# wzf2000/GAMER

Measured on AMD Instinct MI355X. Metric: train-step sequences/sec, Qwen3Multi SMB decoder, his_len=100, higher is better.
Workload: dtype f32 tensors/accumulators, products = 3 x fp16 pieces (split3)

## Files before the change

### gamer_amd/_lib.py

```python
from __future__ import annotations

import ctypes as C
import os
import re
from typing import Optional

import torch

_HERE = os.path.dirname(os.path.abspath(__file__))
LIB_PATH = os.path.join(_HERE, "lib", "libgamer_hip.so")
if os.environ.get("GAMER_LIB_PATH"):
    LIB_PATH = os.path.abspath(os.environ["GAMER_LIB_PATH"])
HEADER_PATH = os.path.join(os.path.dirname(_HERE), "include", "gamer_hip.h")

_lib: Optional[C.CDLL] = None

c_void_p, c_int, c_float, c_int64, c_uint64 = C.c_void_p, C.c_int, C.c_float, C.c_int64, C.c_uint64


class GemmDesc(C.Structure):
    _fields_ = [
        ("A", c_void_p), ("a_rs", c_int64), ("a_ks", c_int64),
        ("B", c_void_p), ("b_rs", c_int64), ("b_ks", c_int64),
        ("C", c_void_p), ("ldc", c_int64),
        ("M", c_int), ("N", c_int), ("K", c_int),
        ("alpha", c_float),
        ("accumulate", c_int),
        ("groups", c_int),
        ("group_mode", c_int),
        ("group_offsets", c_void_p),
        ("strideB", c_int64), ("strideC", c_int64),
        ("kchunk", c_int),
        ("resid", c_void_p),
        ("row_map", c_void_p),
        ("p_drop", c_float),
        ("seed", c_uint64),
        ("rowdot_other", c_void_p),
        ("rowdot_out", c_void_p),
        ("rowdot_S", c_int),
        ("qk_wq", c_void_p), ("qk_wk", c_void_p),
        ("qk_eps", c_float),
        ("qk_cos", c_void_p), ("qk_sin", c_void_p),
        ("qk_bias_q", c_void_p), ("qk_bias_k", c_void_p), ("qk_bias_v", c_void_p),
        ("qk_act_idx", c_void_p),
        ("qk_pos_ids", c_void_p),
        ("qk_q_rot", c_void_p), ("qk_k_rot", c_void_p),
        ("qk_S", c_int), ("qk_nq", c_int), ("qk_nkv", c_int),
        ("b_planes", c_void_p), ("b_plane_stride", c_int64),
        ("amax_a", c_void_p), ("amax_b", c_void_p),
        ("amax_c", c_void_p), ("amax_c_col0", c_int),
        ("wgrad_ws", c_void_p), ("wgrad_ws_floats", c_int64),
        ("sw_gu", c_void_p), ("sw_ld", c_int64),
        ("group_div", c_int), ("sw_tbl", c_void_p), ("b_planes_t", c_void_p),
        ("sw_hm", c_void_p), ("sw_row_group", c_void_p),
    ]


class GemmBf16Desc(C.Structure):
    _fields_ = [
        ("A", c_void_p), ("lda", c_int64),
        ("B", c_void_p), ("ldb", c_int64),
        ("C", c_void_p), ("ldc", c_int64),
        ("M", c_int), ("N", c_int), ("K", c_int),
        ("accumulate", c_int),
        ("groups", c_int),
        ("group_mode", c_int),
        ("group_offsets", c_void_p),
        ("strideB", c_int64), ("strideC", c_int64),
        ("kchunk", c_int),
        ("resid", c_void_p),
        ("row_map", c_void_p),
        ("p_drop", c_float),
        ("seed", c_uint64),
        ("rowdot_other", c_void_p),
        ("rowdot_out", c_void_p),
        ("rowdot_S", c_int),
        ("qk_wq", c_void_p), ("qk_wk", c_void_p), ("qk_eps", c_float),
        ("qk_cos", c_void_p), ("qk_sin", c_void_p),
        ("qk_bias_q", c_void_p), ("qk_bias_k", c_void_p), ("qk_bias_v", c_void_p),
        ("qk_act_idx", c_void_p), ("qk_pos_ids", c_void_p),
        ("qk_q_rot", c_void_p), ("qk_k_rot", c_void_p),
        ("qk_S", c_int), ("qk_nq", c_int), ("qk_nkv", c_int),
        ("sw_gu", c_void_p), ("sw_ld", c_int64),
        ("wgrad_ws", c_void_p), ("wgrad_ws_floats", c_int64),
    ]


P, I, F, L, U = c_void_p, c_int, c_float, c_int64, c_uint64

_SIGNATURES = {
    "gamer_router_fwd": [P, P, P, P, I, I, I, I, I, I, P, P, P, P, P, P, P, P, P, P, P, P],
    "gamer_expert_lists": [P, I, I, I, P, P, P, P, P],
    "gamer_causal_prep": [P, I, I, P, P, P, P, P, P],
    "gamer_session_prep": [P, P, P, I, I, I, I, P, P, P, P, P, P, P],
    "gamer_moe_router_prep": [P, P, P, I, P, I, I, I, I, I, I, I, P, P, P, P, P, P, P, P, P],
    "gamer_embedding_fwd": [P, P, I, I, I, P, P],
    "gamer_embedding_bwd": [P, P, I, I, I, I, P, P],
    "gamer_embedding_bwd_ordered": [P, P, I, I, I, I, P, P, L, P],
    "gamer_embedding_bwd_ordered_ws_bytes": [I, I, I],
    "gamer_rmsnorm_fwd": [P, P, I, I, F, P, P, I, P],
    "gamer_rmsnorm_bwd": [P, P, P, I, P, I, I, F, I, P, P, I, P, P, F, U, P],
    "gamer_colsum_reduce": [P, I, I, I, P, P],
    "gamer_colsum_reduce_batched": [P, L, I, I, I, P, I, P],
    "gamer_rowtable_fwd": [P, P, P, I, I, P, I, I, P],
    "gamer_rowtable_bwd": [P, I, I, P, P, I, I, I, P, P, L, P],
    "gamer_gemm_f32": [C.POINTER(GemmDesc), P],
    "gamer_gemm_f32_split": [C.POINTER(GemmDesc), c_int, P],
    "gamer_split3_guard": [I],
    "gamer_gemm_bf16": [C.POINTER(GemmBf16Desc), P],
    "gamer_cast_params_bf16": [P, P, P, P, I, I, P],
    "gamer_attn_fwd_bf16": [P, I, P, I, P, I, P, P, I, I, I, I, F, F, U, P, P, P, P, P, P, P],
    "gamer_attn_bwd_bf16": [P, I, P, I, P, I, P, P, P, P, P, I, I, I, I, F, F, U, P, P, I, P, I, P, I, P, I, P, P, P, P],
    "gamer_session_spans": [P, P, P, P, P, I, I, I, I, P, P, P, P, P, P, P, P, P],
    "gamer_qknorm_rope_fwd": [P, I, I, I, I, P, P, F, P, P, P, P, P, P, P, P, P, P],
    "gamer_qknorm_rope_bwd": [P, P, P, I, I, I, I, P, P, F, P, P, P, P, P, I, P, P, P, P, P, P, P, P, L, P],
    "gamer_attn_row_order": [P, I, I, P, P, P, P],
    "gamer_attn_fwd": [P, I, P, I, P, I, P, P, P, P, I, I, I, I, F, F, U, P, P, P, P, P, I, P, P],
    "gamer_attn_bwd": [P, I, P, I, P, I, P, P, P, P, P, P, P, I, I, I, I, F, F, U, P, P, I, P, I, P, I, P, P, P, P, P, I, P],
    "gamer_split3_planes": [P, P, L, L, P],
    "gamer_absmax_f32": [P, I, L, I, I, L, P, P],
    "gamer_absmax_multi_f32": [P, P, I, P, P],
    "gamer_split2h_planes_multi": [P, P, I, P, P, P],
    "gamer_amax_sink": [P, P],
    "gamer_amax_sink3": [P, P, P],
    "gamer_attn_split_amax": [P, P, P, P],
    "gamer_attn_fwd_split": [P, I, P, I, P, I, P, P, P, I, I, I, I, F, F, U, P, P, P, P, P, I, P, P],
    "gamer_attn_bwd_split": [P, I, P, I, P, I, P, P, P, P, P, P, P, I, I, I, I, F, F, U, P, P, I, P, I, P, I, P, P, P, I, P, P, P],
    "gamer_residual_dropout_fwd": [P, P, P, I, I, F, U, P, P],
    "gamer_residual_dropout_bwd": [P, P, I, I, F, U, P, P],
    "gamer_swiglu_fwd": [P, P, L, F, U, P, P],
    "gamer_swiglu_bwd": [P, P, P, L, F, U, P],
    "gamer_swiglu_fwd_ld": [P, L, I, I, F, U, P, P],
    "gamer_swiglu_bwd_ld": [P, L, I, I, P, F, U, P],
    "gamer_swiglu_fwd_ld_tbl": [P, L, I, I, F, U, P, P, P, P],
    "gamer_swiglu_bwd_ld_tbl": [P, L, I, I, P, F, U, P, P, P],
    "gamer_silu_fwd_ld": [P, L, I, I, F, U, P, P],
    "gamer_silu_bwd_ld": [P, L, I, I, P, F, U, P],
    "gamer_router_position_table": [P, L, P, I, P],
    "gamer_inject_table_fwd": [P, P, L, I, I, I, I, I, P, P],
    "gamer_segment_colsum_ws_floats": [I, I, I],
    "gamer_segment_colsum": [P, L, I, I, P, I, P, L, P, P],
    "gamer_inject_table_bwd": [P, P, P, L, I, I, I, I, I, P, P, P, P],
    "gamer_silu_gate_fwd": [P, P, L, P, P, F, U, P],
    "gamer_silu_gate_bwd": [P, P, P, L, P, P, F, U, P],
    "gamer_check_labels": [P, L, I, I, P, P],
    "gamer_ce_fwd": [P, I, P, I, I, I, F, I, P, P, P, P, P],
    "gamer_ce_bwd": [P, I, P, I, I, I, F, I, P, P, F, F, P, P],
    "gamer_sumsq": [P, L, P, I, P],
    "gamer_adamw": [P, P, P, P, L, L, F, F, F, F, F, I, F, F, P, I, P, P],
    "gamer_fill_f32": [P, L, F, P],
    "gamer_bias_act_fwd": [P, P, I, I, I, P, P],
    "gamer_bias_act_bwd": [P, P, I, I, I, P, P, I, P],
    "gamer_layernorm_fwd": [P, P, P, P, I, I, F, P, P, P, P, P],
    "gamer_layernorm_bwd": [P, P, P, P, P, I, I, P, P, P, I, P],
    "gamer_attn_dense_fwd": [P, I, P, I, P, I, P, P, I, I, I, I, F, F, U, P, I, P, P],
    "gamer_attn_dense_bwd": [P, I, P, I, P, I, P, P, I, I, I, I, F, F, U, P, P, I, P, P, I, P, I, P, I, P],
    "gamer_reload_env": [],
    "gamer_split2h_transpose_multi": [P, P, I, P, P],
    "gamer_trie_logprobs": [P, L, P, P, P, P, P, I, I, P, P],
    "gamer_trie_advance": [P, P, P, P, P, I, P, P],
    "gamer_kv_append": [P, I, P, I, P, P, I, I, I, I, I, P],
    "gamer_attn_decode": [P, I, P, I, P, I, P, P, P, I, I, I, I, P, I, I, I, I, I, F, P, P],
    "gamer_attn_decode_split": [P, I, P, I, P, I, P, P, P, I, I, I, I, P, I, I, I, I, I, F, P, P, P, P],
    "gamer_catalog_ws_bytes": [I, I, I, I],
    "gamer_catalog_ce_fwd": [P, L, P, I, I, P, I, I, P, P, P, P, P, L, P],
    "gamer_catalog_ce_bwd": [P, L, P, I, I, P, I, I, P, P, P, F, P, P, L, P, L, P],
    "gamer_catalog_topk": [P, L, P, I, I, P, I, I, I, I, I, P, P, P, L, P],
    "gamer_catalog_ce_bias_fwd": [P, L, P, I, I, P, I, I, P, P, P, P, P, P, L, P],
    "gamer_catalog_ce_bias_bwd": [P, L, P, I, I, P, I, I, P, P, P, P, F, P, P, L, P, P, L, P],
    "gamer_catalog_topk_bias": [P, L, P, I, I, P, I, I, P, I, I, I, P, P, P, L, P],
    "gamer_cloze_mask_ws_bytes": [I, I],
    "gamer_cloze_mask": [P, P, I, I, F, F, L, I, U, P, P, P, P, P, P, P, L, P],
    "gamer_embedding_bwd_large_ws_bytes": [I, I, I],
    "gamer_embedding_bwd_large": [P, P, I, I, I, I, P, P, L, P],
    "gamer_position_bwd_ws_floats": [I, I, I],
    "gamer_position_bwd": [P, I, I, I, P, P, L, P],
    "gamer_seq_embed_ln_fwd": [P, P, I, P, I, I, I, P, P, F, F, U, P, P, P, P, P],
    "gamer_gru_gates_floats": [I, I, I],
    "gamer_gru_fwd": [P, P, P, I, I, I, P, P, P],
    "gamer_gru_bwd": [P, P, P, P, P, I, I, I, P, P, P],
    "gamer_mbs_mix_fwd": [P, P, I, I, I, P, P],
    "gamer_mbs_mix_bwd": [P, P, P, I, I, I, P, P, P],
    "gamer_mbs_attn_fwd": [P, I, P, I, P, I, P, P, P, P, P, I, I, I, I, I, I, F, F, U, P, I, P, P],
    "gamer_mbs_attn_bwd": [P, I, P, I, P, I, P, P, P, P, P, I, I, I, I, I, I, F, F, U, P, P, I, P, P, I, P, I, P, I, P, P, P, I, P],
    "gamer_mbs_bias_fold": [P, P, I, I, I, I, P, P],
    "gamer_mbs_gate_mix_fwd": [P, I, P, P, I, I, I, P, P, P],
    "gamer_mbs_gate_mix_bwd": [P, P, P, I, I, I, P, P, I, P],
    "gamer_pbat_attn_fwd": [P, P, P, P, P, P, I, P, P, P, P, P, P, P, P, P, P, P, P, P, P, I, I, I, I, I, F, F, U, P, P, I, P, P, P, P],
    "gamer_pbat_attn_bwd": [P, P, P, P, P, P, I, P, P, P, P, P, P, P, P, P, P, P, P, P, P, I, I, I, I, I, F, F, U, P, P, P, P, I, P, P, P, P, P, P, I, P, P, P, P, I, P, P],
    "gamer_wass_rows_fwd": [P, P, I, I, P, P, P],
    "gamer_wass_rows_bwd": [P, P, P, P, I, I, P, P, P],
    "gamer_wass_table_fwd": [P, P, I, I, P, P, P],
    "gamer_wass_table_bwd": [P, P, P, P, I, I, P, P, P],
    "gamer_rvq_ws_floats": [I],
    "gamer_rvq_fwd": [P, L, P, P, P, I, I, I, I, I, P, P, P, P, P, P, P, P],
    "gamer_rvq_bwd": [P, P, P, P, I, I, I, P, P, F, P, P, P],
    "gamer_msa_linear_fwd": [P, I, P, I, P, I, P, P, P, P, P, I, I, I, I, I, F, F, U, P, I, P, P],
    "gamer_msa_linear_bwd": [P, I, P, I, P, I, P, P, P, P, P, I, I, I, I, I, F, F, U, P, I, P, P, I, P, I, P, I, P, I, P],
    "gamer_seq_mix_fwd": [P, I, P, I, P, I, P, P, I, I, I, P, P],
    "gamer_seq_mix_bwd": [P, I, P, I, P, I, P, P, I, I, I, P, P, P, P, I, P],
    "gamer_hg_build_fwd": [P, P, I, I, I, I, I, P, P, P],
    "gamer_hg_build_bwd": [P, P, P, P, P, I, I, I, I, I, P, P],
    "gamer_hg_conv_fwd": [P, P, I, I, I, P, P],
    "gamer_hg_conv_bwd": [P, P, P, I, I, I, P, P, P],
    "gamer_hg_readout_fwd": [P, P, P, I, I, I, I, I, I, I, P, P],
    "gamer_hg_readout_bwd": [P, P, P, I, I, I, I, I, I, I, P, P],
    "gamer_hg_fuse_fwd": [P, P, P, L, I, P, P, P],
# ... 77 lines not shown
```

### gamer_amd/csrc/common.h

```cpp
#pragma once
#include <hip/hip_runtime.h>
#include <stdint.h>
#include <stdio.h>
#include <stdarg.h>
#include <stdlib.h>
#include <atomic>
#include <type_traits>

#include "../../include/gamer_hip.h"

namespace gamer {

void set_error(const char* fmt, ...);

#define GAMER_CHECK_ARG(cond, ...)                       \
    do {                                                 \
        if (!(cond)) {                                   \
            gamer::set_error(__VA_ARGS__);               \
            return -1;                                   \
        }                                                \
    } while (0)

#define GAMER_CHECK_LAUNCH(name)                                                        \
    do {                                                                                \
// ... 129 lines not shown
AmaxSink take_amax_sink();
void disarm_attn_amax();
__device__ __forceinline__ uint32_t amax_f4(uint32_t m, const float4 v) {
    float f = __uint_as_float(m);
    f = fmaxf(fmaxf(f, fabsf(v.x)), fabsf(v.y));
    f = fmaxf(fmaxf(f, fabsf(v.z)), fabsf(v.w));
    return __float_as_uint(f);
}
constexpr int AMAX_WAYS = 16, AMAX_STRIDE = 16;
__device__ __forceinline__ uint32_t amax_read(const uint32_t* __restrict__ p) {
    uint32_t m = 0;
#pragma unroll
    for (int i = 0; i < AMAX_WAYS; ++i) m = max(m, p[AMAX_STRIDE * i]);
    return m;
}
__device__ __forceinline__ void amax_publish(uint32_t m, uint32_t* __restrict__ out, uint32_t way) {
    uint32_t* w = out + AMAX_STRIDE * (way & (AMAX_WAYS - 1));
    if (m > __hip_atomic_load(w, __ATOMIC_RELAXED, __HIP_MEMORY_SCOPE_AGENT)) atomicMax(w, m);
}
__device__ __forceinline__ void amax_block_commit(uint32_t m, uint32_t* __restrict__ out, uint32_t* __restrict__ lds4) {
    if (!out) return;
#pragma unroll
    for (int o = 32; o > 0; o >>= 1) m = max(m, (uint32_t)__shfl_xor((int)m, o, 64));
    if ((threadIdx.x & 63) == 0) lds4[threadIdx.x >> 6] = m;
    __syncthreads();
    if (threadIdx.x == 0) {
        m = max(max(lds4[0], lds4[1]), max(lds4[2], lds4[3]));
        if (m) amax_publish(m, out, blockIdx.x);
    }
}

__device__ __forceinline__ float wave_sum(float v) {
#pragma unroll
    for (int o = 32; o > 0; o >>= 1) v += __shfl_xor(v, o, 64);
    return v;
}
__device__ __forceinline__ float wave_max(float v) {
#pragma unroll
    for (int o = 32; o > 0; o >>= 1) v = fmaxf(v, __shfl_xor(v, o, 64));
    return v;
}

__device__ __forceinline__ uint32_t mix32(uint32_t x) {
    x ^= x >> 16; x *= 0x7feb352dU; x ^= x >> 15; x *= 0x846ca68bU; x ^= x >> 16;
    return x;
}
struct DropoutRng {
    uint32_t k0, k1, thr;
    float scale;
    bool on;
    __device__ __forceinline__ DropoutRng(float p, uint64_t seed) {
        on = p > 0.f;
        k0 = mix32((uint32_t)seed ^ 0x9e3779b9U);
        k1 = mix32((uint32_t)(seed >> 32) + 0x85ebca6bU);
        float t = p * 4294967296.f;
        thr = t >= 4294967040.f ? 0xffffffffU : (uint32_t)t;
        scale = on ? 1.f / (1.f - p) : 1.f;
    }
    __device__ __forceinline__ void mult4(uint32_t idx4, float (&m)[4]) const {
        if (!on) { m[0] = m[1] = m[2] = m[3] = 1.f; return; }
        const uint32_t thr16 = thr >> 16;
        const uint32_t h1 = mix32(idx4 * 0x9e3779b1U + k0);
        const uint32_t h2 = mix32(h1 ^ k1);
        m[0] = (h1 & 0xffffU) >= thr16 ? scale : 0.f;
        m[1] = (h1 >> 16) >= thr16 ? scale : 0.f;
        m[2] = (h2 & 0xffffU) >= thr16 ? scale : 0.f;
        m[3] = (h2 >> 16) >= thr16 ? scale : 0.f;
    }
    __device__ __forceinline__ float mult(uint64_t idx) const {
        if (!on) return 1.f;
        uint32_t h = mix32((uint32_t)idx ^ k0);
        h = mix32(h + (uint32_t)(idx >> 32) * 0x9e3779b1U + k1);
        return h >= thr ? scale : 0.f;
    }
};

struct AttnDropout {
    uint32_t k0, k1, thr;
    float scale;
    __device__ __forceinline__ AttnDropout(float p, uint64_t seed) {
        k0 = mix32((uint32_t)seed ^ 0x9e3779b9U) ^ mix32((uint32_t)(seed >> 32) + 0x7f4a7c15U);
        k1 = mix32(k0 + 0x632be5abU);
        const float t = p * 4294967296.f;
        thr = t >= 4294967040.f ? 0xffffffffU : (uint32_t)t;
        scale = p > 0.f ? 1.f / (1.f - p) : 1.f;
    }
    __device__ __forceinline__ uint32_t row_word(uint32_t row) const {
        return (mix32(row * 0x9e3779b1U + k0) & 0xffffffU) | 0x800001U;
    }
    __device__ __forceinline__ uint32_t key_word(uint32_t j) const { return mix32(j * 0x85ebca6bU + k1) & 0xffffffU; }
    __device__ __forceinline__ bool keep(uint32_t a, uint32_t b) const { return __umul24(a, b) >= thr; }
};

__device__ __forceinline__ float xor32_max(float v) {
    const auto sw = __builtin_amdgcn_permlane32_swap(__float_as_uint(v), __float_as_uint(v), false, false);
    return fmaxf(__uint_as_float(sw[0]), __uint_as_float(sw[1]));
}
__device__ __forceinline__ float xor32_sum(float v) {
    const auto sw = __builtin_amdgcn_permlane32_swap(__float_as_uint(v), __float_as_uint(v), false, false);
    return __uint_as_float(sw[0]) + __uint_as_float(sw[1]);
}

__device__ __forceinline__ int wave_sum_i32(int v) {
#pragma unroll
    for (int o = 32; o > 0; o >>= 1) v += __shfl_xor(v, o, 64);
    return v;
}
__device__ __forceinline__ int wave_max_i32(int v) {
#pragma unroll
    for (int o = 32; o > 0; o >>= 1) v = max(v, __shfl_xor(v, o, 64));
    return v;
}
__device__ __forceinline__ int wave_min_i32(int v) {
#pragma unroll
    for (int o = 32; o > 0; o >>= 1) v = min(v, __shfl_xor(v, o, 64));
    return v;
}

#define GAMER_DPP_ROW_REDUCE(OP, v)                                                                   \
    v = OP(v, __builtin_amdgcn_update_dpp(v, v, 0xB1, 0xf, 0xf, false));      \
    v = OP(v, __builtin_amdgcn_update_dpp(v, v, 0x4E, 0xf, 0xf, false));      \
    v = OP(v, __builtin_amdgcn_update_dpp(v, v, 0x141, 0xf, 0xf, false));         \
    v = OP(v, __builtin_amdgcn_update_dpp(v, v, 0x140, 0xf, 0xf, false));
__device__ __forceinline__ int wave_min_i32_dpp(int v) {
    GAMER_DPP_ROW_REDUCE(min, v)
    return min(min(__builtin_amdgcn_readlane(v, 0), __builtin_amdgcn_readlane(v, 16)),
               min(__builtin_amdgcn_readlane(v, 32), __builtin_amdgcn_readlane(v, 48)));
}
__device__ __forceinline__ int wave_max_i32_dpp(int v) {
    GAMER_DPP_ROW_REDUCE(max, v)
    return max(max(__builtin_amdgcn_readlane(v, 0), __builtin_amdgcn_readlane(v, 16)),
               max(__builtin_amdgcn_readlane(v, 32), __builtin_amdgcn_readlane(v, 48)));
}

__device__ __forceinline__ float row16_sum_dpp(float v) {
#define GAMER_DPP_F(ctrl) __int_as_float(__builtin_amdgcn_update_dpp(__float_as_int(v), __float_as_int(v), ctrl, 0xf, 0xf, false))
    v += GAMER_DPP_F(0xB1);
    v += GAMER_DPP_F(0x4E);
    v += GAMER_DPP_F(0x141);
    v += GAMER_DPP_F(0x140);
#undef GAMER_DPP_F
    return v;
}

__device__ __forceinline__ float sigmoid_f(float x) { return __builtin_amdgcn_rcpf(1.f + __expf(-x)); }
__device__ __forceinline__ float silu_f(float x) { return x * sigmoid_f(x); }
__device__ __forceinline__ float dsilu_f(float x) {
    const float s = sigmoid_f(x);
    return s * (1.f + x * (1.f - s));
}

bool gemm_as_eligible(const gamer_gemm_desc* d, bool a_kc, bool b_kc, const uint16_t* b_planes);
int launch_gemm_as(const gamer_gemm_desc* d, const uint16_t* b_planes, bool b_kc, hipStream_t st);
bool gemm_os_eligible(const gamer_gemm_desc* d, bool a_kc, bool b_kc, const uint16_t* b_planes);
int launch_gemm_os(const gamer_gemm_desc* d, const uint16_t* b_planes, int guard, hipStream_t st, bool fwd_t = false);
bool gemm_os_fwd_eligible(const gamer_gemm_desc* d, bool a_kc, bool b_kc);
bool gemm_wg_eligible(const gamer_gemm_desc* d, bool a_kc, bool b_kc);
int launch_gemm_wg(const gamer_gemm_desc* d, hipStream_t st);

int launch_wgrad_reduce(const float* ws, float* C, int64_t ldc, int M, int N, int groups, const int32_t* group_offsets, int K,
                        int kchunk, int64_t strideC, hipStream_t st);

}
```

### gamer_amd/csrc/gemm.hip

```cpp
#include "common.h"
#include <stdlib.h>

namespace gamer {

constexpr int BM = 128, BN = 128, BK = 32;
constexpr int GEMM_THREADS = 256;
constexpr int KC_LD = BK + 4;
constexpr int TILE_FLOATS = BM * KC_LD;
constexpr int GEMM_LDS_BYTES = 4 * TILE_FLOATS * (int)sizeof(float);

typedef float f32x16 __attribute__((ext_vector_type(16)));

constexpr int SP_KC_ROW = 80;
constexpr int SP_KC_IMG = BM * SP_KC_ROW;
constexpr int SP_RC_IMG = BK * 256;
constexpr int SP_OPERAND = 3 * SP_KC_IMG;
constexpr int SP_LDS_BYTES = 2 * SP_OPERAND;

#ifndef SP_ABLATE
#define SP_ABLATE 0
#endif
__device__ __forceinline__ uint32_t pack_hi16(uint32_t w0, uint32_t w1) { return __builtin_amdgcn_perm(w1, w0, 0x07060302u); }
__device__ __forceinline__ void split3(float x, uint32_t (&w)[3]) {
    if (SP_ABLATE & 1) { w[0] = w[1] = w[2] = __float_as_uint(x); return; }
// ... 1212 lines not shown
    const int64_t step4 = (int64_t)tiles_mn * (BM * BN) / 4;
    float4 s = make_float4(0.f, 0.f, 0.f, 0.f);
    int c = 0;
    for (; c + 4 <= c_n; c += 4) {
        const float4 a0 = src[(int64_t)c * step4], a1 = src[(int64_t)(c + 1) * step4], a2 = src[(int64_t)(c + 2) * step4],
                     a3 = src[(int64_t)(c + 3) * step4];
        s.x = (((s.x + a0.x) + a1.x) + a2.x) + a3.x; s.y = (((s.y + a0.y) + a1.y) + a2.y) + a3.y;
        s.z = (((s.z + a0.z) + a1.z) + a2.z) + a3.z; s.w = (((s.w + a0.w) + a1.w) + a2.w) + a3.w;
    }
    for (; c < c_n; ++c) {
        const float4 a0 = src[(int64_t)c * step4];
        s.x += a0.x; s.y += a0.y; s.z += a0.z; s.w += a0.w;
    }
    const int row = (tile / n_tiles) * BM + lr, col = (tile % n_tiles) * BN + lc;
    if (row < M && c_n > 0) {
        float* dst = C + (int64_t)g * strideC + (int64_t)row * ldc + col;
        const float v[4] = {s.x, s.y, s.z, s.w};
#pragma unroll
        for (int e = 0; e < 4; ++e)
            if (col + e < N) dst[e] += v[e];
    }
}

int launch_wgrad_reduce(const float* ws, float* C, int64_t ldc, int M, int N, int groups, const int32_t* group_offsets, int K,
                        int kchunk, int64_t strideC, hipStream_t st) {
    const int m_tiles = (M + BM - 1) / BM, n_tiles = (N + BN - 1) / BN;
    const int64_t rblocks = (int64_t)groups * m_tiles * n_tiles * 16;
    hipLaunchKernelGGL(wgrad_reduce_kernel, dim3((int)rblocks), dim3(256), 0, st, ws, C, ldc, M, N, m_tiles, n_tiles, groups,
                       group_offsets, K, kchunk, strideC);
    return (int)hipGetLastError();
}

__global__ void __launch_bounds__(256)
split3_planes_kernel(const float4* __restrict__ x, uint16_t* __restrict__ planes, int64_t n4, int64_t stride) {
    for (int64_t i = (int64_t)blockIdx.x * 256 + threadIdx.x; i < n4; i += (int64_t)gridDim.x * 256) {
        uint2 img[3];
        split3_quad(x[i], img);
#pragma unroll
        for (int s = 0; s < 3; ++s) *reinterpret_cast<uint2*>(planes + s * stride + 4 * i) = img[s];
    }
}

}

using namespace gamer;

extern "C" int gamer_split3_planes(const float* x, gamer_bf16* planes, int64_t n, int64_t plane_stride, void* stream) {
    GAMER_CHECK_ARG(x && planes && n > 0 && n % 4 == 0 && plane_stride >= n && plane_stride % 4 == 0 && aligned16(x) &&
                    (reinterpret_cast<uintptr_t>(planes) & 7u) == 0,
                    "gamer_split3_planes: n=%lld and plane_stride=%lld must be multiples of 4 (stride >= n), x 16-byte and planes 8-byte aligned",
                    (long long)n, (long long)plane_stride);
    const int64_t n4 = n / 4;
    int blocks = (int)((n4 + 255) / 256);
    if (blocks > 4096) blocks = 4096;
    hipLaunchKernelGGL(split3_planes_kernel, dim3(blocks), dim3(256), 0, (hipStream_t)stream, reinterpret_cast<const float4*>(x),
                       reinterpret_cast<uint16_t*>(planes), n4, plane_stride);
    GAMER_CHECK_LAUNCH("gamer_split3_planes");
    return 0;
}

extern "C" int gamer_debug_gemm_stamp(void* p) {
    unsigned long long* v = (unsigned long long*)p;
    return (int)hipMemcpyToSymbol(HIP_SYMBOL(g_gemm_stamp), &v, sizeof(v));
}

static inline bool diag_build_switches() {
    static EnvSwitch stamp("GAMER_GEMM_STAMP"), nbuf("GAMER_GEMM_NBUF");
    return stamp.is_set() || nbuf.is_set();
}
static inline bool diag_pp_switch() { static EnvSwitch pp("GAMER_GEMM_PP"); return pp.is_set(); }
static int gemm_entry(const gamer_gemm_desc* d, void* stream, int split) {
    GAMER_CHECK_ARG(d, "gamer_gemm_f32: null descriptor");
    GAMER_CHECK_ARG(d->A && d->B && d->C, "gamer_gemm_f32: null matrix pointer");
    GAMER_CHECK_ARG(d->M > 0 && d->N > 0 && d->K > 0, "gamer_gemm_f32: bad shape M=%d N=%d K=%d", d->M, d->N, d->K);
    GAMER_CHECK_ARG((d->a_rs == 1) != (d->a_ks == 1) || (d->a_rs == 1 && d->a_ks == 1 && (d->M == 1 || d->K == 1)),
                    "gamer_gemm_f32: exactly one of a_rs/a_ks must be 1 (rs=%lld ks=%lld)", (long long)d->a_rs, (long long)d->a_ks);
    GAMER_CHECK_ARG((d->b_rs == 1) != (d->b_ks == 1) || (d->b_rs == 1 && d->b_ks == 1 && (d->N == 1 || d->K == 1)),
                    "gamer_gemm_f32: exactly one of b_rs/b_ks must be 1 (rs=%lld ks=%lld)", (long long)d->b_rs, (long long)d->b_ks);
    const bool a_kc = d->a_ks == 1, b_kc = d->b_ks == 1;
    const int64_t a_ld = a_kc ? d->a_rs : d->a_ks, b_ld = b_kc ? d->b_rs : d->b_ks;
    GAMER_CHECK_ARG(a_ld % 4 == 0 && b_ld % 4 == 0 && d->ldc >= d->N,
                    "gamer_gemm_f32: leading dims must be multiples of 4 (lda=%lld ldb=%lld ldc=%lld)",
                    (long long)a_ld, (long long)b_ld, (long long)d->ldc);
    GAMER_CHECK_ARG(aligned16(d->A) && aligned16(d->B), "gamer_gemm_f32: A and B must be 16-byte aligned");
    GAMER_CHECK_ARG(d->groups >= 1 && (d->groups == 1 || d->group_offsets), "gamer_gemm_f32: groups=%d needs group_offsets", d->groups);
    GAMER_CHECK_ARG(d->strideB % 4 == 0, "gamer_gemm_f32: strideB must be a multiple of 4");
    GAMER_CHECK_ARG(d->group_mode == 0 || d->group_mode == 1, "gamer_gemm_f32: group_mode=%d", d->group_mode);

    GemmParams p;
    p.A = d->A; p.a_rs = d->a_rs; p.a_ks = d->a_ks;
    p.B = d->B; p.b_rs = d->b_rs; p.b_ks = d->b_ks;
    p.C = d->C; p.ldc = d->ldc;
    p.M = d->M; p.N = d->N; p.K = d->K;
    p.alpha = d->alpha; p.accumulate = d->accumulate;
    p.groups = d->groups; p.group_offsets = d->group_offsets;
    p.strideB = d->strideB; p.strideC = d->strideC;
    p.kchunk = d->kchunk;
    p.resid = d->resid; p.row_map = d->row_map; p.p_drop = d->p_drop; p.seed = d->seed;
    p.rowdot_other = d->rowdot_other; p.rowdot_out = d->rowdot_out; p.rowdot_S = d->rowdot_S;
    p.qk_wq = d->qk_wq; p.qk_wk = d->qk_wk; p.qk_eps = d->qk_eps; p.qk_cos = d->qk_cos; p.qk_sin = d->qk_sin;
    p.qk_bias_q = d->qk_bias_q; p.qk_bias_k = d->qk_bias_k; p.qk_bias_v = d->qk_bias_v;
    p.qk_act_idx = d->qk_act_idx; p.qk_pos_ids = d->qk_pos_ids; p.qk_q_rot = d->qk_q_rot; p.qk_k_rot = d->qk_k_rot;
    p.qk_S = d->qk_S; p.qk_nq = d->qk_nq; p.qk_nkv = d->qk_nkv;
    p.amax_a = d->amax_a; p.amax_b = d->amax_b;
    p.guard = g_split3_guard;
    p.amax_c = d->amax_c; p.amax_c_col0 = d->amax_c_col0;
    p.wgrad_ws = nullptr;
    p.sw_gu = d->sw_gu; p.sw_ld = d->sw_ld;
    p.group_div = d->group_div > 1 ? d->group_div : 1; p.sw_tbl = d->sw_tbl;
    GAMER_CHECK_ARG(d->group_div <= 1 || (d->group_mode == 0 && d->group_offsets && d->groups % d->group_div == 0),
                    "gamer_gemm_f32: group_div = %d needs group_mode 0, group_offsets and groups (%d) a multiple of it", d->group_div, d->groups);
    GAMER_CHECK_ARG(!d->sw_tbl || ((d->sw_gu || d->sw_hm) && aligned16(d->sw_tbl)),
                    "gamer_gemm_f32: sw_tbl is an option of the SwiGLU epilogues (sw_gu, sw_hm)");
    GAMER_CHECK_ARG(!d->sw_gu || (split == 3 && d->group_mode == 0 && !d->accumulate && !d->resid && !d->rowdot_out && !d->qk_q_rot &&
                                  d->alpha == 1.f && d->N % 4 == 0 && d->sw_ld >= 2 * (int64_t)d->N && d->sw_ld % 4 == 0 &&
                                  aligned16(d->sw_gu) && d->p_drop >= 0.f && d->p_drop < 1.f),
                    "gamer_gemm_f32: the SwiGLU-backward epilogue (sw_gu) is built for gamer_gemm_f32_split(terms = 3), a plain input-"
                    "gradient GEMM with alpha = 1, N %% 4 == 0, sw_ld >= 2 N (N=%d sw_ld=%lld)", d->N, (long long)d->sw_ld);
    GAMER_CHECK_ARG(!d->amax_c || (d->group_mode == 0 && !d->accumulate && !d->resid && !d->qk_q_rot && d->amax_c_col0 >= 0 &&
                                   d->amax_c_col0 % 64 == 0),
                    "gamer_gemm_f32: amax_c needs a plain or row-dot Linear-forward / input-gradient GEMM (no accumulate, residual or "
                    "q|k|v epilogue) and amax_c_col0 a multiple of 64 (amax_c_col0=%d)", d->amax_c_col0);
    GAMER_CHECK_ARG(split != 3 || (d->amax_a && d->amax_b), "gamer_gemm_f32_split: terms = 3 needs amax_a and amax_b (gamer_absmax_f32)");
    p.b_planes = (split && d->group_mode == 0) ? (const uint16_t*)d->b_planes : nullptr;
    p.b_plane_stride = d->b_plane_stride;
    GAMER_CHECK_ARG(!p.b_planes || split == 3 || ((reinterpret_cast<uintptr_t>(p.b_planes) & 7u) == 0 && d->b_plane_stride % 4 == 0 && d->b_plane_stride > 0),
                    "gamer_gemm_f32_split: b_planes must be 8-byte aligned with b_plane_stride %% 4 == 0");
    GAMER_CHECK_ARG(!p.b_planes || split != 3 || (reinterpret_cast<uintptr_t>(p.b_planes) & 15u) == 0,
                    "gamer_gemm_f32_split: terms = 3 takes b_planes as packed pieces at B's offsets (16-byte aligned)");
    if (split == 3 && p.b_planes && ((b_kc ? d->K : d->N) % 4) != 0) p.b_planes = nullptr;
    GAMER_CHECK_ARG(!d->qk_q_rot || (d->qk_k_rot && d->qk_wq && d->qk_wk && d->qk_cos && d->qk_sin && d->group_mode == 0 &&
                                     d->groups == 1 && a_kc && b_kc && !d->resid && !d->rowdot_out && !d->accumulate &&
                                     d->alpha == 1.f && d->M % BM == 0 && d->qk_nq > 0 && d->qk_nkv > 0 && d->qk_S > 0 &&
                                     d->N == (d->qk_nq + 2 * d->qk_nkv) * 64 && d->N % BN == 0 && d->ldc % 4 == 0 &&
                                     aligned16(d->C) && aligned16(d->qk_q_rot) && aligned16(d->qk_k_rot) &&
                                     (!d->qk_bias_q || (d->qk_bias_k && d->qk_bias_v && d->qk_act_idx)) &&
                                     !diag_build_switches()),
                    "gamer_gemm_f32: the q|k|v epilogue needs a Linear-forward layout, one group, M %% 128 == 0 (M=%d), "
                    "N = (nq + 2 nkv) * 64 a multiple of 128 (N=%d), alpha = 1 and no other epilogue", d->M, d->N);
    GAMER_CHECK_ARG(!d->rowdot_out || (d->rowdot_other && d->rowdot_S > 0 && d->group_mode == 0 && d->groups == 1 &&
                                       !d->resid && !d->accumulate && d->M % BM == 0 && d->N % BN == 0 &&
                                       d->M % d->rowdot_S == 0 && d->ldc % 4 == 0 && aligned16(d->rowdot_other) &&
                                       aligned16(d->C) && !diag_build_switches()),
                    "gamer_gemm_f32: the row-dot epilogue needs full 128 x 128 tiles (M=%d N=%d), one group, ldc %% 4 == 0",
                    d->M, d->N);
    GAMER_CHECK_ARG(!d->resid || (d->group_mode == 0 && !d->accumulate && a_kc && b_kc && d->ldc % 4 == 0 &&
                                  aligned16(d->resid) && aligned16(d->C) && d->p_drop >= 0.f && d->p_drop < 1.f),
                    "gamer_gemm_f32: the fused residual epilogue needs a Linear-forward layout, ldc %% 4 == 0, no accumulate");
    GAMER_CHECK_ARG(!d->sw_hm || (d->group_mode == 0 && a_kc && b_kc && !d->accumulate && !d->resid && !d->rowdot_out && !d->qk_q_rot &&
                                  !d->sw_gu && d->alpha == 1.f && d->N % 8 == 0 && d->ldc >= d->N && d->ldc % 4 == 0 && aligned16(d->sw_hm) &&
                                  aligned16(d->C) && (!d->sw_tbl || d->sw_row_group) && d->p_drop >= 0.f && d->p_drop < 1.f),
                    "gamer_gemm_f32: the SwiGLU-forward epilogue (sw_hm) needs a Linear-forward layout with N = 2 I (N=%d), alpha = 1, no other "
                    "epilogue, and sw_row_group with sw_tbl", d->N);
    if (split == 3 && gemm_as_eligible(d, a_kc, b_kc, p.b_planes)) return launch_gemm_as(d, p.b_planes, b_kc, (hipStream_t)stream);
    if (d->sw_hm) {
        gamer_gemm_desc d2 = *d;
        d2.sw_hm = nullptr; d2.sw_row_group = nullptr; d2.sw_tbl = nullptr; d2.amax_c = nullptr;
        const int rc = gemm_entry(&d2, stream, split);
        if (rc) return rc;
        if (d->amax_c) gamer_amax_sink(d->amax_c, nullptr);
        return d->sw_tbl ? gamer_swiglu_fwd_ld_tbl(d->C, d->ldc, d->M, d->N / 2, d->p_drop, d->seed, d->sw_hm, d->sw_tbl, d->sw_row_group, stream)
                         : gamer_swiglu_fwd_ld(d->C, d->ldc, d->M, d->N / 2, d->p_drop, d->seed, d->sw_hm, stream);
    }
    if (split == 3 && gemm_os_eligible(d, a_kc, b_kc, p.b_planes)) return launch_gemm_os(d, p.b_planes, g_split3_guard, (hipStream_t)stream);
    if (split == 3 && gemm_os_fwd_eligible(d, a_kc, b_kc))
        return launch_gemm_os(d, reinterpret_cast<const uint16_t*>(d->b_planes_t), g_split3_guard, (hipStream_t)stream, true);
    p.n_tiles = (d->N + BN - 1) / BN;
    hipStream_t st = (hipStream_t)stream;

    if (d->group_mode == 0) {
        p.m_tiles = (d->M + BM - 1) / BM + (d->group_offsets ? d->groups : 0);
        const int64_t blocks = (int64_t)p.m_tiles * p.n_tiles;
        GAMER_CHECK_ARG(blocks < (1LL << 31), "gamer_gemm_f32: grid too large");
        if (a_kc && b_kc) return launch_gemm<true, true, 0>(p, (int)blocks, st, split);
        if (a_kc && !b_kc) return launch_gemm<true, false, 0>(p, (int)blocks, st, split);
        if (!a_kc && !b_kc) return launch_gemm<false, false, 0>(p, (int)blocks, st, split);
        GAMER_CHECK_ARG(false, "gamer_gemm_f32: layout (A row-contiguous, B k-contiguous) is not built");
    } else {
        GAMER_CHECK_ARG(!a_kc && !b_kc, "gamer_gemm_f32: group_mode 1 (wgrad) needs row-contiguous A and B");
        GAMER_CHECK_ARG(d->kchunk >= BK && d->kchunk % BK == 0, "gamer_gemm_f32: kchunk=%d must be a positive multiple of 32", d->kchunk);
        p.m_tiles = (d->M + BM - 1) / BM;
        const int64_t chunks = (d->K + d->kchunk - 1) / d->kchunk + (d->group_offsets ? d->groups : 0);
        const int64_t blocks = chunks * p.m_tiles * p.n_tiles;
        GAMER_CHECK_ARG(blocks < (1LL << 31), "gamer_gemm_f32: grid too large");
        p.wgrad_ws = d->wgrad_ws;
        if (p.wgrad_ws) {
            const int64_t need = chunks * p.m_tiles * p.n_tiles * (int64_t)(BM * BN);
            GAMER_CHECK_ARG(d->wgrad_ws_floats >= need && aligned16(d->wgrad_ws),
                            "gamer_gemm_f32: wgrad_ws holds %lld floats, this weight gradient needs %lld (chunks x tiles x 16384)",
                            (long long)d->wgrad_ws_floats, (long long)need);
            GAMER_CHECK_ARG(!diag_pp_switch(), "gamer_gemm_f32: the deterministic weight gradient is not built for the ping-pong form");
        }
        const int rc = (split == 3 && p.wgrad_ws && gemm_wg_eligible(d, a_kc, b_kc)) ? launch_gemm_wg(d, st)
                                                                                     : launch_gemm<false, false, 1>(p, (int)blocks, st, split);
        if (rc || !p.wgrad_ws) return rc;
        const int64_t rblocks = (int64_t)d->groups * p.m_tiles * p.n_tiles * 16;
        hipLaunchKernelGGL(wgrad_reduce_kernel, dim3((int)rblocks), dim3(256), 0, st, p.wgrad_ws, d->C, d->ldc, d->M, d->N, p.m_tiles,
                           p.n_tiles, d->groups, d->group_offsets, d->K, d->kchunk, d->strideC);
        GAMER_CHECK_LAUNCH("gamer_gemm_f32/wgrad_reduce");
        return 0;
    }
    return 0;
}

__device__ __forceinline__ uint32_t amax4(uint32_t m, const uint4 v) {
    return max(max(m, v.x & 0x7fffffffu), max(max(v.y & 0x7fffffffu, v.z & 0x7fffffffu), v.w & 0x7fffffffu));
}
__device__ __forceinline__ void amax_commit(uint32_t m, uint32_t* __restrict__ out) {
    __shared__ uint32_t part[4];
#pragma unroll
    for (int o = 32; o > 0; o >>= 1) m = max(m, (uint32_t)__shfl_xor((int)m, o, 64));
    if ((threadIdx.x & 63) == 0) part[threadIdx.x >> 6] = m;
    __syncthreads();
    if (threadIdx.x == 0) {
        m = max(max(part[0], part[1]), max(part[2], part[3]));
        if (m) amax_publish(m, out, blockIdx.x);
    }
}
__global__ void __launch_bounds__(256)
absmax_flat_kernel(const uint4* __restrict__ x, int64_t n4, uint32_t* __restrict__ out) {
    uint32_t m = 0;
    const int64_t step = (int64_t)gridDim.x * 256;
    int64_t i = (int64_t)blockIdx.x * 256 + threadIdx.x;
    for (; i + step < n4; i += 2 * step) {
        const uint4 a = x[i], b = x[i + step];
        m = amax4(amax4(m, a), b);
    }
    if (i < n4) m = amax4(m, x[i]);
    amax_commit(m, out);
}
__global__ void __launch_bounds__(256)
absmax_rows_kernel(const float* __restrict__ x, int batch, int64_t stride, int rows, int cols, int64_t ld, uint32_t* __restrict__ out) {
    const int lane = threadIdx.x & 63;
    const int64_t waves = (int64_t)gridDim.x * 4, nrows = (int64_t)batch * rows;
    uint32_t m = 0;
    for (int64_t w = (int64_t)blockIdx.x * 4 + (threadIdx.x >> 6); w < nrows; w += waves) {
        const int64_t b = w / rows, r = w - b * rows;
        const float* src = x + b * stride + r * ld;
        for (int c = lane << 2; c < cols; c += 256) {
            if (c + 3 < cols) m = amax4(m, *reinterpret_cast<const uint4*>(src + c));
            else for (int q = 0; c + q < cols; ++q) m = max(m, __float_as_uint(src[c + q]) & 0x7fffffffu);
        }
    }
    amax_commit(m, out);
}
extern "C" int gamer_absmax_f32(const float* x, int batch, int64_t stride, int rows, int cols, int64_t ld, uint32_t* out, void* stream) {
    GAMER_CHECK_ARG(x && out && batch >= 1 && rows >= 1 && cols >= 1 && ld >= cols && ld % 4 == 0 && stride % 4 == 0 &&
                    (reinterpret_cast<uintptr_t>(x) & 15u) == 0, "gamer_absmax_f32: bad arguments (rows=%d cols=%d ld=%lld)",
                    rows, cols, (long long)ld);
    if (ld == cols && (batch == 1 || stride == (int64_t)rows * ld)) {
        const int64_t n4 = (int64_t)batch * rows * cols / 4;
        int64_t blocks = (n4 + 511) / 512;
        if (blocks < 1) blocks = 1;
        if (blocks > 2048) blocks = 2048;
        hipLaunchKernelGGL(absmax_flat_kernel, dim3((int)blocks), dim3(256), 0, (hipStream_t)stream,
                           reinterpret_cast<const uint4*>(x), n4, out);
    } else {
        int64_t blocks = ((int64_t)batch * rows + 3) / 4;
        if (blocks > 2048) blocks = 2048;
        hipLaunchKernelGGL(absmax_rows_kernel, dim3((int)blocks), dim3(256), 0, (hipStream_t)stream, x, batch, stride, rows, cols, ld, out);
    }
    GAMER_CHECK_LAUNCH("gamer_absmax_f32");
    return 0;
}

__global__ void __launch_bounds__(256)
absmax_multi_kernel(const float* __restrict__ base, const int64_t* __restrict__ table, int bpe, uint32_t* __restrict__ out) {
    const int e = blockIdx.x / bpe, part = blockIdx.x % bpe;
    const uint4* x = reinterpret_cast<const uint4*>(base + table[2 * e]);
    const int64_t n4 = table[2 * e + 1] >> 2;
    uint32_t m = 0;
    for (int64_t i = (int64_t)part * 256 + threadIdx.x; i < n4; i += (int64_t)bpe * 256) m = amax4(m, x[i]);
    __shared__ uint32_t part4[4];
#pragma unroll
    for (int o = 32; o > 0; o >>= 1) m = max(m, (uint32_t)__shfl_xor((int)m, o, 64));
    if ((threadIdx.x & 63) == 0) part4[threadIdx.x >> 6] = m;
    __syncthreads();
    if (threadIdx.x == 0) {
        m = max(max(part4[0], part4[1]), max(part4[2], part4[3]));
        if (m) amax_publish(m, out + (int64_t)e * 256, (uint32_t)part);
    }
}
extern "C" int gamer_absmax_multi_f32(const float* base, const int64_t* table, int n, uint32_t* out, void* stream) {
    GAMER_CHECK_ARG(base && table && out && n >= 1 && (reinterpret_cast<uintptr_t>(base) & 15u) == 0, "gamer_absmax_multi_f32: bad arguments");
    const int bpe = 16;
    hipLaunchKernelGGL(absmax_multi_kernel, dim3(n * bpe), dim3(256), 0, (hipStream_t)stream, base, table, bpe, out);
    GAMER_CHECK_LAUNCH("gamer_absmax_multi_f32");
    return 0;
}

__global__ void __launch_bounds__(256)
split2h_planes_multi_kernel(const float* __restrict__ base, const int64_t* __restrict__ table, int bpe,
                            const uint32_t* __restrict__ slots, uint16_t* __restrict__ planes) {
    const int e = blockIdx.x / bpe, part = blockIdx.x % bpe;
    const int64_t off = table[2 * e], n4 = table[2 * e + 1] >> 2;
    float s, inv;
    scale_from_amax(amax_read(slots + (int64_t)e * 256), s, inv);
    const float4* x = reinterpret_cast<const float4*>(base + off);
    for (int64_t i = (int64_t)part * 256 + threadIdx.x; i < n4; i += (int64_t)bpe * 256) {
        uint2 img[2];
        split2h_quad(x[i], s, img);
        reinterpret_cast<uint4*>(planes)[(off >> 2) + i] = make_uint4(img[0].x, img[0].y, img[1].x, img[1].y);
    }
}
extern "C" int gamer_split2h_planes_multi(const float* base, const int64_t* table, int n, const uint32_t* slots, gamer_bf16* planes,
                                          void* stream) {
    GAMER_CHECK_ARG(base && table && slots && planes && n >= 1 && (reinterpret_cast<uintptr_t>(base) & 15u) == 0 &&
// ... 50 lines not shown
```

### gamer_amd/csrc/gemm_as.hip

```cpp
#include "common.h"
#include <stdlib.h>
#include <atomic>

namespace gamer {

typedef float f32x16 __attribute__((ext_vector_type(16)));
typedef uint32_t u32x4a __attribute__((ext_vector_type(4)));

#ifndef AS_WAVES
#define AS_WAVES 4
#endif
#ifndef AS_NT
#define AS_NT 1
#endif
#ifndef AS_DEPTH
#define AS_DEPTH 1
#endif
#ifndef AS_ABLATE
#define AS_ABLATE 0
#endif
constexpr int AS_SLAB = 32 * AS_NT;
constexpr int AS_PANEL = AS_SLAB * 64;

__device__ __forceinline__ int as_f(int row) { return (((row >> 1) & 1) << 2) | (((row >> 3) & 1) << 1) | ((row >> 2) & 1); }
__device__ __forceinline__ int as_off(int row, int col) { return row * 64 + ((((col >> 3) ^ as_f(row))) << 3) + (col & 7); }

struct AsParams {
    const float* A; int64_t lda;
    const uint16_t* Wp;
    int64_t ldw;
    float* C; int64_t ldc;
    int M, N, K;
    float alpha;
    const uint32_t* amax_w;
    uint32_t* amax_c; int amax_c_col0;
    int groups; const int32_t* group_offsets; int64_t strideW;
    int accumulate;
    const float* rowdot_other; float* rowdot_out; int rowdot_S;
    float* sw_gu; int64_t sw_ld; float p_drop; uint64_t seed;
    float* hm; const float* tbl; int group_div;
};

template <int KP, bool WRC, int EPI, int NW>
__global__ void __launch_bounds__(64 * NW, AS_DEPTH == 2 ? 1 : 8 / NW)
gemm_as_kernel(const AsParams p) {
    constexpr int AS_WAVES_K = NW, AS_THREADS_K = 64 * NW;
    extern __shared__ __attribute__((aligned(16))) unsigned char as_raw[];
    bf16_t* const wimg = reinterpret_cast<bf16_t*>(as_raw);
    __shared__ uint32_t amax_word;
    const int tid = threadIdx.x, lane = tid & 63, w = tid >> 6;
    const int r = lane & 31, h = lane >> 5;
    int row0 = blockIdx.x * (32 * AS_WAVES_K), row_end = p.M, grp = 0;
    if (p.group_offsets) {
        int prev = p.group_offsets[0], tiles_before = 0;
        bool found = false;
        for (int gi = 0; gi < p.groups; ++gi) {
            const int nxt = p.group_offsets[gi + 1];
            const int tiles = (nxt - prev + 32 * AS_WAVES_K - 1) / (32 * AS_WAVES_K);
            if (!found && (int)blockIdx.x < tiles_before + tiles) {
                grp = gi; row0 = prev + ((int)blockIdx.x - tiles_before) * (32 * AS_WAVES_K); row_end = nxt; found = true;
            }
            if (!found) tiles_before += tiles;
            prev = nxt;
        }
        if (!found) return;
    }
    const int m = row0 + w * 32 + r;
    const bool valid_m = m < row_end;
    if (tid == 0) amax_word = 0;

    bf16x8 af[2][KP * 4];
    float row_inv;
    {
        const float* arow = p.A + (int64_t)(valid_m ? m : row_end - 1) * p.lda + 8 * h;
        float4 raw[KP * 8];
#pragma unroll
        for (int s = 0; s < KP * 4; ++s) {
            raw[2 * s] = *reinterpret_cast<const float4*>(arow + 16 * s);
            raw[2 * s + 1] = *reinterpret_cast<const float4*>(arow + 16 * s + 4);
        }
        float mx = 0.f;
#pragma unroll
        for (int i = 0; i < KP * 8; ++i) {
            if (!valid_m) raw[i] = make_float4(0.f, 0.f, 0.f, 0.f);
            mx = fmaxf(fmaxf(fmaxf(mx, fabsf(raw[i].x)), fabsf(raw[i].y)), fmaxf(fabsf(raw[i].z), fabsf(raw[i].w)));
        }
        mx = xor32_max(mx);
        float s_row = 1.f;
        row_inv = 1.f;
        if (mx > 0.f) scale_from_amax(__float_as_uint(mx), s_row, row_inv);
#pragma unroll
        for (int s = 0; s < KP * 4; ++s) {
            u32x4a u0, u1;
#pragma unroll
            for (int j = 0; j < 2; ++j) {
                const float4 x = raw[2 * s + j];
                uint32_t a0, a1, b0, b1;
                cut2h_quad(x.x, x.y, x.z, x.w, s_row, a0, a1, b0, b1);
                u0[2 * j] = a0; u0[2 * j + 1] = b0; u1[2 * j] = a1; u1[2 * j + 1] = b1;
            }
            af[0][s] = __builtin_bit_cast(bf16x8, u0);
            af[1][s] = __builtin_bit_cast(bf16x8, u1);
        }
    }
    float w_s, w_inv;
    scale_from_amax(amax_read(p.amax_w), w_s, w_inv);
    const float out_scale = row_inv * w_inv * p.alpha;

    const int n_slabs = (p.N + AS_SLAB - 1) / AS_SLAB;
    constexpr int QPR = KP * 16;
    constexpr int NLD = AS_SLAB * QPR / AS_THREADS_K;
    uint4 rw[NLD], rw2[NLD];
    int lds_off[NLD], nl_[NLD];
    const uint4* wsrc[NLD];
#pragma unroll
    for (int i = 0; i < NLD; ++i) {
        const int f = tid + AS_THREADS_K * i;
        if (!WRC) {
            const int nl = f / QPR, g = f % QPR;
            nl_[i] = nl;
            lds_off[i] = (g >> 4) * AS_PANEL + as_off(nl, (4 * g) & 63);
            wsrc[i] = reinterpret_cast<const uint4*>(p.Wp) + (((int64_t)(grp / p.group_div) * p.strideW + (int64_t)nl * p.ldw + 4 * g) >> 2);
        } else {
            const int k = f / (AS_SLAB / 4), nq = f % (AS_SLAB / 4);
            nl_[i] = 4 * nq;
            lds_off[i] = k * AS_SLAB + 4 * nq;
            wsrc[i] = reinterpret_cast<const uint4*>(p.Wp) + (((int64_t)(grp / p.group_div) * p.strideW + (int64_t)k * p.ldw + 4 * nq) >> 2);
        }
    }
    const int64_t slab_stride = WRC ? (AS_SLAB >> 2) : (((int64_t)AS_SLAB * p.ldw) >> 2);
    auto load_slab_into = [&](int j, uint4 (&dst)[NLD]) {
        const bool full = (j + 1) * AS_SLAB <= p.N;
#pragma unroll
        for (int i = 0; i < NLD; ++i) {
            const uint4* src = wsrc[i] + (int64_t)j * slab_stride;
            if (!full && j * AS_SLAB + nl_[i] >= p.N) src = wsrc[i];
            dst[i] = *src;
        }
    };
    auto store_slab_from = [&](int j, int buf, const uint4 (&rw)[NLD]) {
        bf16_t* img = wimg + buf * (2 * KP * AS_PANEL);
        const bool full = (j + 1) * AS_SLAB <= p.N;
#pragma unroll
        for (int i = 0; i < NLD; ++i) {
            const bool ok = full || j * AS_SLAB + nl_[i] < p.N;
            *reinterpret_cast<uint2*>(img + lds_off[i]) = ok ? make_uint2(rw[i].x, rw[i].y) : make_uint2(0u, 0u);
            *reinterpret_cast<uint2*>(img + KP * AS_PANEL + lds_off[i]) = ok ? make_uint2(rw[i].z, rw[i].w) : make_uint2(0u, 0u);
        }
    };
    auto load_slab = [&](int j) { load_slab_into(j, rw); };
    auto store_slab = [&](int j, int buf) { store_slab_from(j, buf, rw); };
    int row_off[4];
#pragma unroll
    for (int s = 0; s < 4; ++s) row_off[s] = as_off(r, 16 * s + 8 * h);
    const int tr_lane = (8 * h + ((lane >> 2) & 3)) * AS_SLAB + 16 * ((lane >> 4) & 1) + 4 * (lane & 3);
    auto read_tr = [&](const bf16_t* base) -> bf16x8 {
        bf16x8 out;
#pragma unroll
        for (int c = 0; c < 2; ++c) {
            const bf16x4 v = __builtin_amdgcn_ds_read_tr16_b64_v4bf16((bf16x4 __attribute__((address_space(3)))*)(base + c * 4 * AS_SLAB));
            out[4 * c + 0] = v[0]; out[4 * c + 1] = v[1]; out[4 * c + 2] = v[2]; out[4 * c + 3] = v[3];
        }
        return out;
    };
    float hd_dot = 0.f;
    float emax = 0.f;
    float4 gsave[EPI == 5 ? 4 * AS_NT : 1];
    float* const tbl_lds = reinterpret_cast<float*>(as_raw + (size_t)(AS_DEPTH == 2 ? 3 : 2) * 2 * KP * AS_PANEL * sizeof(bf16_t));
    if (EPI == 5 && p.tbl) {
        const float4* src = reinterpret_cast<const float4*>(p.tbl + (int64_t)grp * p.N);
        for (int i = tid; i < p.N / 4; i += AS_THREADS_K) reinterpret_cast<float4*>(tbl_lds)[i] = src[i];
    }

    float cmax = 0.f;
    float* crow = p.C + (int64_t)m * p.ldc;
    f32x16 acc[AS_NT];
    auto mfma_slab = [&](const int j, const int buf) {
        const bf16_t* img = wimg + buf * (2 * KP * AS_PANEL);
#pragma unroll
            for (int i = 0; i < 16; ++i)
#pragma unroll
                for (int nt = 0; nt < AS_NT; ++nt) acc[nt][i] = 0.f;
#pragma unroll
            for (int ks = 0; ks < KP * 4; ++ks) {
                const int pn = ks >> 2, s = ks & 3;
#pragma unroll
                for (int nt = 0; nt < AS_NT; ++nt) {
                    bf16x8 w0, w1;
                    if (!WRC) {
                        w0 = *reinterpret_cast<const bf16x8*>(img + pn * AS_PANEL + nt * 32 * 64 + row_off[s]);
                        w1 = *reinterpret_cast<const bf16x8*>(img + (KP + pn) * AS_PANEL + nt * 32 * 64 + row_off[s]);
                    } else {
                        w0 = read_tr(img + ks * 16 * AS_SLAB + nt * 32 + tr_lane);
                        w1 = read_tr(img + KP * AS_PANEL + ks * 16 * AS_SLAB + nt * 32 + tr_lane);
                    }
                    if (AS_ABLATE & 2) { asm volatile("" :: "v"(w0), "v"(w1)); continue; }
                    acc[nt] = __builtin_amdgcn_mfma_f32_32x32x16_f16(__builtin_bit_cast(f16x8, w1), __builtin_bit_cast(f16x8, af[0][ks]), acc[nt], 0, 0, 0);
                    acc[nt] = __builtin_amdgcn_mfma_f32_32x32x16_f16(__builtin_bit_cast(f16x8, w0), __builtin_bit_cast(f16x8, af[1][ks]), acc[nt], 0, 0, 0);
                    acc[nt] = __builtin_amdgcn_mfma_f32_32x32x16_f16(__builtin_bit_cast(f16x8, w0), __builtin_bit_cast(f16x8, af[0][ks]), acc[nt], 0, 0, 0);
                }
            }
    };
    auto epilogue_slab = [&](const int j) {
            float part = 0.f;
            if (valid_m) {
                const bool track = EPI != 5 && p.amax_c != nullptr && j * AS_SLAB >= p.amax_c_col0;
#pragma unroll
                for (int nt = 0; nt < AS_NT; ++nt)
#pragma unroll
                    for (int g4 = 0; g4 < 4; ++g4) {
                        const int col = j * AS_SLAB + nt * 32 + 8 * g4 + 4 * h;
                        if (col < p.N) {
                            float4 t4 = make_float4(acc[nt][4 * g4] * out_scale, acc[nt][4 * g4 + 1] * out_scale,
                                                    acc[nt][4 * g4 + 2] * out_scale, acc[nt][4 * g4 + 3] * out_scale);
                            if (AS_ABLATE & 1) { asm volatile("" :: "v"(t4.x), "v"(t4.y), "v"(t4.z), "v"(t4.w)); continue; }
                            if (EPI == 4) {
                                float* ga = p.sw_gu + (int64_t)m * p.sw_ld + col;
                                const float4 a4 = *reinterpret_cast<const float4*>(ga), b4 = *reinterpret_cast<const float4*>(ga + p.N);
                                const DropoutRng rng(p.p_drop, p.seed);
                                float mu[4];
                                rng.mult4((uint32_t)(((int64_t)m * p.N + col) >> 2), mu);
                                const float d0 = mu[0] * t4.x, d1 = mu[1] * t4.y, d2 = mu[2] * t4.z, d3 = mu[3] * t4.w;
                                const float4 dg = make_float4(d0 * b4.x * dsilu_f(a4.x), d1 * b4.y * dsilu_f(a4.y), d2 * b4.z * dsilu_f(a4.z),
                                                              d3 * b4.w * dsilu_f(a4.w));
                                const float4 du = make_float4(d0 * silu_f(a4.x), d1 * silu_f(a4.y), d2 * silu_f(a4.z), d3 * silu_f(a4.w));
                                *reinterpret_cast<float4*>(ga) = dg;
                                *reinterpret_cast<float4*>(ga + p.N) = du;
                                emax = fmaxf(fmaxf(fmaxf(emax, fmaxf(fabsf(dg.x), fabsf(du.x))), fmaxf(fabsf(dg.y), fabsf(du.y))),
                                             fmaxf(fmaxf(fabsf(dg.z), fabsf(du.z)), fmaxf(fabsf(dg.w), fabsf(du.w))));
                                continue;
                            }
                            if (p.accumulate) {
                                const float4 o = *reinterpret_cast<const float4*>(crow + col);
                                t4.x += o.x; t4.y += o.y; t4.z += o.z; t4.w += o.w;
                            }
                            if (col + 4 <= p.N) {
                                *reinterpret_cast<float4*>(crow + col) = t4;
                            } else {
                                const float e[4] = {t4.x, t4.y, t4.z, t4.w};
                                for (int q = 0; q < 4 && col + q < p.N; ++q) crow[col + q] = e[q];
                            }
                            if (EPI == 2) {
                                const float4 o4 = *reinterpret_cast<const float4*>(p.rowdot_other + (int64_t)m * p.ldc + col);
                                part += (t4.x * o4.x + t4.y * o4.y) + (t4.z * o4.z + t4.w * o4.w);
                            }
                            if (EPI == 5) {
                                const int half = p.N >> 1;
                                float4 x4 = t4;
                                if (p.tbl) {
                                    const float4 tb = *reinterpret_cast<const float4*>(tbl_lds + col);
                                    x4.x += tb.x; x4.y += tb.y; x4.z += tb.z; x4.w += tb.w;
                                }
                                if (col < half) {
                                    gsave[EPI == 5 ? nt * 4 + g4 : 0] = x4;
                                } else {
                                    const float4 g = gsave[EPI == 5 ? nt * 4 + g4 : 0];
                                    const int hc = col - half;
                                    const DropoutRng rng(p.p_drop, p.seed);
                                    float mu[4];
                                    rng.mult4((uint32_t)(((int64_t)m * half + hc) >> 2), mu);
                                    const float4 o = make_float4(mu[0] * (silu_f(g.x) * x4.x), mu[1] * (silu_f(g.y) * x4.y),
                                                                 mu[2] * (silu_f(g.z) * x4.z), mu[3] * (silu_f(g.w) * x4.w));
                                    *reinterpret_cast<float4*>(p.hm + (int64_t)m * half + hc) = o;
                                    emax = fmaxf(fmaxf(fmaxf(emax, fabsf(o.x)), fabsf(o.y)), fmaxf(fabsf(o.z), fabsf(o.w)));
                                }
                            }
                            if (track) cmax = fmaxf(fmaxf(fmaxf(cmax, fabsf(t4.x)), fabsf(t4.y)), fmaxf(fabsf(t4.z), fabsf(t4.w)));
                        }
                    }
            }
            if (EPI == 2) {
                const float sl = xor32_sum(part);
                constexpr int SPH = 64 / AS_SLAB;
                hd_dot = (j % SPH == 0) ? sl : hd_dot + sl;
                if (j % SPH == SPH - 1 && valid_m && h == 0) {
                    const int heads = p.N >> 6, head = (j * AS_SLAB) >> 6;
                    p.rowdot_out[((int64_t)(m / p.rowdot_S) * heads + head) * p.rowdot_S + m % p.rowdot_S] = hd_dot;
                }
            }
    };
    if (AS_DEPTH == 1) {
        load_slab(0);
        store_slab(0, 0);
        __syncthreads();
        auto slab_of = [&](int i) { return EPI == 5 ? (i >> 1) + (i & 1) * (n_slabs >> 1) : i; };
#pragma unroll 1
        for (int i = 0; i < n_slabs; ++i) {
            const int j = slab_of(i), buf = i & 1, jn = slab_of(min(i + 1, n_slabs - 1));
            if (!(AS_ABLATE & 4)) load_slab(jn);
            __builtin_amdgcn_sched_barrier(0);
            mfma_slab(j, buf);
            __builtin_amdgcn_sched_barrier(0);
            if (!(AS_ABLATE & 4)) store_slab(jn, buf ^ 1);
            epilogue_slab(j);
            __syncthreads();
        }
    } else {
        load_slab_into(0, rw);
        store_slab_from(0, 0, rw);
        if (n_slabs > 1) load_slab_into(1, rw);
        if (n_slabs > 2) load_slab_into(2, rw2);
        __syncthreads();
        int bufc = 0;
#pragma unroll 1
        for (int j = 0; j < n_slabs; j += 2) {
            const int b1 = bufc == 2 ? 0 : bufc + 1, b2 = b1 == 2 ? 0 : b1 + 1;
            mfma_slab(j, bufc); epilogue_slab(j);
            if (j + 1 < n_slabs) store_slab_from(j + 1, b1, rw);
            if (j + 3 < n_slabs) load_slab_into(j + 3, rw);
            __syncthreads();
            if (j + 1 >= n_slabs) break;
            mfma_slab(j + 1, b1); epilogue_slab(j + 1);
            if (j + 2 < n_slabs) store_slab_from(j + 2, b2, rw2);
            if (j + 4 < n_slabs) load_slab_into(j + 4, rw2);
            __syncthreads();
            bufc = b2;
        }
    }
    if (p.amax_c) {
        uint32_t mw = __float_as_uint((EPI == 4 || EPI == 5) ? emax : cmax);
#pragma unroll
        for (int o2 = 32; o2 > 0; o2 >>= 1) mw = max(mw, (uint32_t)__shfl_xor((int)mw, o2, 64));
        if (lane == 0 && mw) atomicMax(&amax_word, mw);
        __syncthreads();
        if (tid == 0 && amax_word) amax_publish(amax_word, p.amax_c, blockIdx.x);
    }
}

static std::atomic<long long> g_as_launches{0};

static inline bool gemm_as_enabled() {
    static EnvSwitch sw("GAMER_GEMM_AS");
    return sw.get(1) != 0;
}

bool gemm_as_eligible(const gamer_gemm_desc* d, bool a_kc, bool b_kc, const uint16_t* b_planes) {
    if (!gemm_as_enabled() || !a_kc || !b_planes || !d->amax_b) return false;
    if (d->group_mode != 0 || d->resid || d->qk_q_rot) return false;
    if ((d->group_div > 1 || d->sw_tbl) && !d->sw_hm) return false;
    if (d->sw_hm) {
        static EnvSwitch sw5("GAMER_GEMM_AS_SWIGLU");
        if (sw5.get(1) == 0 || !b_kc || d->accumulate || d->rowdot_out || d->sw_gu || d->N % (2 * AS_SLAB) != 0 || d->alpha != 1.f ||
            !aligned16(d->sw_hm) || (d->sw_tbl && (!aligned16(d->sw_tbl) || !d->group_offsets)) || d->p_drop < 0.f || d->p_drop >= 1.f)
            return false;
        if (d->group_div > 1 && (!d->group_offsets || d->groups % d->group_div != 0)) return false;
    }
    static EnvSwitch min_m("GAMER_GEMM_AS_MIN_M");
    if (d->K % 64 != 0 || d->K < 64 || d->K > 256 || d->M < min_m.get(16384)) return false;
    if (d->a_rs % 4 != 0 || d->ldc % 4 != 0 || !aligned16(d->C) || !aligned16(b_planes)) return false;
    if (d->groups != 1 && (!d->group_offsets || d->strideC != 0)) return false;
    if (d->groups == 1 && d->group_offsets) return false;
    if (b_kc) {
        if (d->accumulate || d->rowdot_out || d->sw_gu || d->b_rs % 4 != 0) return false;
        if (d->groups != 1 && d->amax_c && !d->sw_hm) return false;
        if (d->amax_c && !d->sw_hm && d->amax_c_col0 % AS_SLAB != 0) return false;
        return true;
    }
    static EnvSwitch rc("GAMER_GEMM_AS_RC");
    const int rc_mode = rc.get(1);
    if (rc_mode == 0) return false;
    if (d->K != 256 || d->N % 4 != 0 || d->b_ks % 4 != 0) return false;
    if ((d->sw_gu || d->rowdot_out) && rc_mode < 2) return false;
    if (d->sw_gu) {
        return !d->amax_c || d->amax_c_col0 == 0;
    }
    if (d->groups != 1) return false;
    if (d->rowdot_out) return !d->accumulate && d->N % 64 == 0 && 64 % AS_SLAB == 0 && (!d->amax_c || d->amax_c_col0 % AS_SLAB == 0);
    return !d->amax_c || (!d->accumulate && d->amax_c_col0 % AS_SLAB == 0);
}

template <int KP, bool WRC, int EPI>
static int launch_as(int nw, dim3 grid, size_t shmem, hipStream_t st, const AsParams& p) {
    const char* who = "gamer_gemm_f32_split/activation-stationary";
    if constexpr (EPI == 5) return launch<gemm_as_kernel<KP, WRC, EPI, 4>>(who, grid, dim3(64 * 4), shmem, st, p);
    else
        return with_flags([&](auto eight) { return launch<gemm_as_kernel<KP, WRC, EPI, eight() ? 8 : 4>>(who, grid, dim3(eight() ? 512 : 256), shmem, st, p); },
                          nw == 8);
}

int launch_gemm_as(const gamer_gemm_desc* d, const uint16_t* b_planes, bool b_kc, hipStream_t st) {
    AsParams p;
    p.A = d->A; p.lda = d->a_rs;
    p.Wp = b_planes; p.ldw = b_kc ? d->b_rs : d->b_ks;
    p.C = d->C; p.ldc = d->ldc;
    p.M = d->M; p.N = d->N; p.K = d->K;
    p.alpha = d->alpha;
    p.amax_w = d->amax_b;
    p.amax_c = d->amax_c; p.amax_c_col0 = d->amax_c_col0;
    p.groups = d->groups; p.group_offsets = d->groups > 1 ? d->group_offsets : nullptr; p.strideW = d->strideB;
    p.accumulate = d->accumulate;
    p.rowdot_other = d->rowdot_other; p.rowdot_out = d->rowdot_out; p.rowdot_S = d->rowdot_S;
    p.sw_gu = d->sw_gu; p.sw_ld = d->sw_ld; p.p_drop = d->p_drop; p.seed = d->seed;
    p.hm = d->sw_hm; p.tbl = d->sw_hm ? d->sw_tbl : nullptr; p.group_div = d->group_div > 1 ? d->group_div : 1;
    const int kp = d->K / 64;
    const size_t shmem = (size_t)(AS_DEPTH == 2 ? 3 : 2) * 2 * kp * AS_PANEL * sizeof(bf16_t) + (d->sw_hm ? (size_t)d->N * sizeof(float) : 0);
    static EnvSwitch wv("GAMER_GEMM_AS_WAVES");
    const int nw = d->sw_hm ? 4 : (wv.is_set() ? (wv.get(4) == 8 ? 8 : 4) : ((b_kc && d->groups == 1 && d->N >= 512 && AS_WAVES == 4) ? 8 : AS_WAVES));
    const dim3 grid((d->M + 32 * nw - 1) / (32 * nw) + (p.group_offsets ? d->groups : 0));
    int rc;
    if (b_kc && d->sw_hm) {
        switch (kp) {
            case 1: rc = launch_as<1, false, 5>(nw, grid, shmem, st, p); break;
            case 2: rc = launch_as<2, false, 5>(nw, grid, shmem, st, p); break;
            case 3: rc = launch_as<3, false, 5>(nw, grid, shmem, st, p); break;
            default: rc = launch_as<4, false, 5>(nw, grid, shmem, st, p); break;
        }
    } else if (b_kc) {
        switch (kp) {
            case 1: rc = launch_as<1, false, 0>(nw, grid, shmem, st, p); break;
            case 2: rc = launch_as<2, false, 0>(nw, grid, shmem, st, p); break;
            case 3: rc = launch_as<3, false, 0>(nw, grid, shmem, st, p); break;
            default: rc = launch_as<4, false, 0>(nw, grid, shmem, st, p); break;
        }
    } else if (d->sw_gu) {
        rc = launch_as<4, true, 4>(nw, grid, shmem, st, p);
    } else if (d->rowdot_out) {
        rc = launch_as<4, true, 2>(nw, grid, shmem, st, p);
    } else {
        rc = launch_as<4, true, 0>(nw, grid, shmem, st, p);
    }
    if (rc) return rc;
    g_as_launches.fetch_add(1, std::memory_order_relaxed);
    return 0;
}

}

extern "C" long long gamer_debug_gemm_as_launches(void) { return gamer::g_as_launches.load(std::memory_order_relaxed); }
```

### gamer_amd/engine.py

```python
from __future__ import annotations

import contextlib
import functools
import math
import os
from types import SimpleNamespace
from typing import Dict, List, Optional, Tuple

import torch

from . import ops
from .config import Qwen3MultiConfig

IGNORE_INDEX = -100


def _round_up(x: int, m: int) -> int:
    return (x + m - 1) // m * m


class _FlatLayout:

    def __init__(self, decay: List[Tuple[str, tuple]], nodecay: List[Tuple[str, tuple]]):
        self.entries: Dict[str, Tuple[int, tuple]] = {}
# ... 391 lines not shown
        self.ordered_embedding_grad = os.environ.get("GAMER_EMBEDDING_ATOMICS", "0") == "0"
        self._check_deterministic_embedding()
        self._saved = None

    def _check_deterministic_embedding(self):
        V = self.cfg.vocab_size
        if self.ordered_embedding_grad and V > 8191 and self.deterministic:
            raise RuntimeError(f"Engine(deterministic=True): the ordered embedding gradient takes at most 8191 vocabulary rows (V = {V}); "
                               "the float-atomics scatter it would fall back to is not reproducible")

    def init_weights(self, seed: int = 0):
        g = torch.Generator(device="cpu").manual_seed(seed)
        std = self.cfg.initializer_range
        for name, (off, shp) in self.layout.entries.items():
            n = math.prod(shp)
            if len(shp) == 1:
                self.flat_p[off:off + n].fill_(1.0)
            else:
                self.flat_p[off:off + n].copy_(torch.randn(n, generator=g) * std)
        self.params["model.embed_tokens.weight"][self.cfg.pad_token_id].zero_()

    def load_state_dict(self, sd: Dict[str, torch.Tensor]):
        missing = [k for k in self.layout.entries if k not in sd]
        if missing:
            raise KeyError(f"missing parameters: {missing[:5]}{'...' if len(missing) > 5 else ''}")
        for k, p in self.params.items():
            if tuple(sd[k].shape) != tuple(p.shape):
                raise ValueError(f"{k}: shape {tuple(sd[k].shape)} != {tuple(p.shape)}")
            p.copy_(sd[k].to(torch.float32))

    def rope(self, S: int):
        if S not in self._rope:
            dh, theta = self.cfg.head_dim, float(self.cfg.rope_theta)
            inv_freq = 1.0 / (theta ** (torch.arange(0, dh, 2, dtype=torch.int64).to(torch.float32) / dh))
            freqs = torch.arange(S, dtype=torch.float32)[:, None] * inv_freq[None, :]
            emb = torch.cat((freqs, freqs), dim=-1)
            self._rope[S] = (emb.cos().to(self.device).contiguous(), emb.sin().to(self.device).contiguous())
        return self._rope[S]

    def workspace(self, B: int, S: int, train: bool) -> _Workspace:
        if train not in self._ws:
            spill = not (self.split_attention and self.matmul != "f32" and
                         (not self.key_spans or (self.matmul == "split3" and self.h2_attention)))
            self._ws[train] = _Workspace(self.cfg, self.device, train, self.act_dtype, spill, self._bind_masks)
        return self._ws[train].bind(B, S)

    @staticmethod
    def _bind_masks(ws: _Workspace, B: int, S: int):
        i32 = torch.int32
        T, E, n_t32 = B * S, ws.cfg.num_experts, (S + 31) // 32
        buf = ws._buf
        ws.router = {k: buf("r_" + k, (B, S), i32) for k in
                     ("expert", "beh_idx", "act_idx", "kl_self", "kl_cross", "ql_cross", "empty_self", "empty_cross")}
        ws.router["tile_empty_self"] = buf("r_tile_empty_self", (B, n_t32), i32)
        ws.router["tile_empty_cross"] = buf("r_tile_empty_cross", (B, n_t32), i32)
        if "r_bad_token" not in ws._store:
            ws._store["r_bad_token"] = torch.zeros(1, dtype=i32, device=ws.device)
        ws.router["bad_token"] = ws._store["r_bad_token"]
        ws.session = None
        ws.perm = buf("perm", (T,), i32)
        ws.slot = buf("slot", (T,), i32)
        ws.cross_order = (buf("co_perm", (B, S), i32), buf("co_kind", (B, n_t32), i32), buf("co_maxpos", (B, n_t32), i32))
        ws.offsets = buf("offsets", (E + 1,), i32)
        ws.work = buf("work", ((B + 1) * E,), i32)

    def reserve(self, B: int, S: int, train: bool = True):
        self.workspace(B, S, train)

    def _seed(self, layer: int, site: int) -> int:
        return ((self.base_seed & 0xFFFF) << 48) | ((self.dropout_step & 0xFFFFFFFF) << 16) | (layer << 4) | site

    def _planes(self):
        wp = self.weight_planes
        return None if wp is None else (self.flat_p.data_ptr(), self.flat_p.numel() * 4, wp.data_ptr(), wp.stride(0))

    @ops.scoped_f32_matmul(lambda self, *a: self.matmul, lambda self, *a: self._planes())
    @ops.scoped_amax(lambda self, *a: self._amax)
    def forward(self, input_ids, attention_mask=None, actions=None, labels=None, num_items_in_batch=None,
                train: bool = False, dropout: Optional[bool] = None, act_zero_col: Optional[int] = None,
                uniform_len: int = 0, kv_sink=None, kv_dest=None, session_ids=None, extended_session_ids=None,
                last_row_logits: bool = False, hidden_sink: Optional[list] = None, rope_from_mask: bool = False):
        cfg = self.cfg
        B, S = input_ids.shape
        if train and self._item_aligned and S % cfg.num_positions != 0:
            raise ValueError(f"sequence length {S} is not a multiple of num_positions={cfg.num_positions} "
                             "(the router assumes item-aligned sequences, router.py:78-81)")
        if train and (act_zero_col is not None or uniform_len not in (0, S) or rope_from_mask):
            raise ValueError("act_zero_col / uniform_len / rope_from_mask are evaluation-only options")
        c = self._prologue(input_ids, attention_mask, labels, train, dropout, cfg.dropout_rate, kv_dest, hidden_sink,
                           last_row_logits, uniform_len,
                           eval_only="last_row_logits is an evaluation-only option" if last_row_logits else None,
                           f32_only=("generation (cached decode / re-run scoring) is built for dtype='f32' only"
                                     if last_row_logits or uniform_len not in (0, S) else None))
        ws, ids, am, bf16 = c.ws, c.ids, c.am, c.bf16
        T, H, nq, nkv, I, E = c.T, c.H, c.nq, c.nkv, c.I, cfg.num_experts
        NQ, NKV, QKV, eps, scale, cos, sin, p_res = c.NQ, c.NKV, c.QKV, c.eps, c.scale, c.cos, c.sin, c.p_res
        r = ws.router
        r["bad_token"].zero_()
        pos_ids = self._route(c, actions, act_zero_col, rope_from_mask)
        NB1 = cfg.num_behavior + 1
        if self.split_inject:
            ws.grp_key = ws._buf("grp_key", (B, S), torch.int32)
            ws.grp_offsets = ws._buf("grp_offsets", (E * NB1 + 1,), torch.int32)
            ws.row_group = ws._buf("row_group", (T,), torch.int32)
            torch.add(r["beh_idx"], r["expert"], alpha=NB1, out=ws.grp_key)
            ops.expert_lists(ws.grp_key, E * NB1, ws.perm, ws.slot, ws.grp_offsets, ws._buf("grp_work", ((B + 1) * E * NB1,), torch.int32))
            ws.offsets.copy_(ws.grp_offsets[::NB1])
            torch.index_select(ws.grp_key.view(-1), 0, ws.perm, out=ws.row_group)
            if self._amax is not None:
                self._amax.register(*[self.W[l].gu for l in cfg.behavior_injection_decoder])
        else:
            ops.expert_lists(r["expert"], E, ws.perm, ws.slot, ws.offsets, ws.work)
        if self._amax is not None and self._amax.planes_t is not None:
            for Wl in self.W:
                self._amax.register_transposed(Wl.self_attn["o"], 1, H, NQ)
                self._amax.register_transposed(Wl.down, Wl.ne, H, I)
                if Wl.cross:
                    self._amax.register_transposed(Wl.cross_attn["o"], 1, H, NQ)
        span_self = span_cross = None
        if self.variant == "session":
            if session_ids is None:
                raise ValueError("Session IDs must be provided to generate session-wise causal mask.")
            sid = session_ids.to(self.device, torch.int64).contiguous()
            ext = (extended_session_ids.to(self.device, torch.int64).contiguous()
                   if extended_session_ids is not None else None)
            if ws.session is None:
                i32 = torch.int32
                if "s_violations" not in ws._store:
                    ws._store["s_violations"] = torch.zeros(1, dtype=i32, device=self.device)
                ws.session = {"span_self": ws._buf("s_span_self", (B, S, 4), i32),
                              "span_cross": ws._buf("s_span_cross", (B, S, 4), i32),
                              "pos_ids": ws._buf("s_pos_ids", (B, S), i32), "violations": ws._store["s_violations"]}
            ws.session["violations"].zero_()
            ops.session_spans(sid, ext, am, cfg.num_positions, S, r, ws.session)
            span_self, span_cross, pos_ids = (ws.session["span_self"], ws.session["span_cross"],
                                              ws.session["pos_ids"])
        if cfg.cross_attention_decoder:
            ops.attn_row_order(r["empty_cross"], *ws.cross_order)
        ops.embedding_fwd(ids, self.params["model.embed_tokens.weight"], ws.x[0][0])

        fuse_qkv = ((self.fuse_qkv_bf16 if bf16 else self.fuse_qkv) and ops.qkv_fused_ok(ws.layers[0]["h1"], T, QKV)
                    and cfg.head_dim == 64)
        attention = functools.partial(self._attention, c)

        for l in range(cfg.num_hidden_layers):
            W, A, xs = self.W[l], ws.layers[l], ws.x[l]
            Wm = self.Wm[l]
            if hidden_sink is not None:
                hidden_sink.append(xs[0].view(B, S, H).clone())
            self._self_attention(c, l, r, span_self, pos_ids, fuse_qkv, kv_dest, kv_sink)
            xcur = xs[1]
            if W.cross:
                C, Cm = W.cross_attn, Wm.cross_attn
                ops.rmsnorm_fwd(xs[1], W.ln2, eps, A["h2"])
                qkv_x, k_x = kv_dest(l, "cross") if kv_dest is not None else (A["qkv_c"], A["k_c"])
                h2_hold = self._amax.hold(A["h2"]) if (self._amax is not None and not train) else None
                if h2_hold is not None:
                    h2_hold.__enter__()
                if fuse_qkv:
                    ops.gemm(A["h2"], H, 1, Cm["qkv"], H, 1, qkv_x, QKV, T, QKV, H,
                             qknorm=dict(wq=C["qn"], wk=C["kn"], eps=eps, cos=cos, sin=sin, q_rot=A["q_c"], k_rot=k_x,
                                         bias_q=C["bq"], bias_k=C["bk"], bias_v=C["bv"], act_idx=r["act_idx"],
                                         pos_ids=pos_ids, S=S, nq=nq, nkv=nkv))
                else:
                    ops.linear_fwd(A["h2"], H, Cm["qkv"], H, qkv_x, QKV, T, QKV, H)
                    ops.qknorm_rope_fwd(qkv_x, S, nq, nkv, C["qn"], C["kn"], eps, cos, sin, A["q_c"], k_x,
                                        bias_q=C["bq"], bias_k=C["bk"], bias_v=C["bv"], act_idx=r["act_idx"],
                                        pos_ids=pos_ids)
                if kv_sink is not None:
                    kv_sink(l, "cross", k_x, qkv_x[:, NQ + NKV:])
                if (last_row_logits and l == cfg.num_hidden_layers - 1 and span_cross is None and not bf16 and
                        os.environ.get("GAMER_PREFILL_LAST_ROW", "1") != "0"):
                    rows = torch.arange(B, device=self.device) * S + (S - 1)
                    f32 = dict(dtype=torch.float32, device=self.device)
                    q_l = A["q_c"].index_select(0, rows).contiguous()
                    key_ok = (r["kl_cross"].view(B, S) < r["ql_cross"].view(B, S)[:, S - 1:S]).to(torch.int32).contiguous()
                    uni = (r["empty_cross"].view(B, S)[:, S - 1] != 0).to(torch.int32).contiguous()
                    kg0 = torch.zeros(B, 1, NKV, **f32)
                    ao_l = torch.empty(B, NQ, **f32)
                    ops.attn_decode(q_l, k_x, qkv_x[:, NQ + NKV:], key_ok, kg0, kg0, 0, False, uni, B, 1, S, nq, nkv, scale, ao_l)
                    op_l, gate_l, x_cross_last = torch.empty(B, H, **f32), torch.empty(B, H, **f32), torch.empty(B, H, **f32)
                    ops.linear_fwd(ao_l, NQ, Cm["o"], NQ, op_l, H, B, H, NQ)
                    ops.linear_fwd(A["h2"].index_select(0, rows).contiguous(), H, Cm["gate"], H, gate_l, H, B, H, H)
                    ops.silu_gate_fwd(op_l, gate_l, x_cross_last, resid=xs[1].index_select(0, rows).contiguous())
                    xcur = None
                else:
                    x_cross_last = None
                    attention(A["q_c"], k_x, qkv_x[:, NQ + NKV:], r["kl_cross"], r["ql_cross"], r["empty_cross"],
                              r["tile_empty_cross"], self._seed(l, 2), A["ao_c"], A["lse_c"], ws.cross_order, span_cross)
                if x_cross_last is None:
                    ops.linear_fwd(A["ao_c"], NQ, Cm["o"], NQ, A["op_c"], H, T, H, NQ)
                    ops.linear_fwd(A["h2"], H, Cm["gate"], H, A["gate_c"], H, T, H, H)
                if h2_hold is not None:
                    h2_hold.__exit__(None, None, None)
                if x_cross_last is None:
                    ops.silu_gate_fwd(A["op_c"], A["gate_c"], xs[2], resid=xs[1], p=p_res, seed=self._seed(l, 3))
                    xcur = xs[2]
            din = W.din
            if last_row_logits and l == cfg.num_hidden_layers - 1:
                rows = torch.arange(B, device=self.device) * S + (S - 1)
                xl = x_cross_last if (W.cross and x_cross_last is not None) else xcur.index_select(0, rows).contiguous()
                f32 = dict(dtype=torch.float32, device=self.device)
                beh = r["beh_idx"].view(-1).index_select(0, rows).contiguous() if W.inject else None
                x_last = torch.empty(B, H, **f32)
                self.ffn_rows(W, (S - 1) % cfg.num_positions, xl, beh, x_last)
                break
            xnext = ws.x[l + 1][0] if l + 1 < cfg.num_hidden_layers else ws.x_final
            if not self._shipped_ffn_layer(W):
                self._ffn_fwd_plain(c, l, xcur, xnext)
                continue
            grp = dict(groups=E, group_offsets=ws.offsets)
            if W.inject and self.split_inject:
                hin = A["hin"].view(-1)[:T * H].view(T, H)
                ops.rmsnorm_fwd(xcur, W.ln3, eps, hin, H, ws.slot)
                tb = ws._buf((f"l{l}_" if train else "l_") + "inject_tbl", (E * NB1, 2 * I))
                ops.inject_table_fwd(W.beh, W.gu, din, H, E, 2 * I, tb)
                if c.fuse_swiglu_fwd:
                    ops.gemm(hin, H, 1, Wm.gu, din, 1, A["gu"], 2 * I, T, 2 * I, H, strideB=2 * I * din, groups=E * NB1,
                             group_offsets=ws.grp_offsets, group_div=NB1, p_drop=p_res, seed=self._seed(l, 4),
                             swiglu_fwd=(A["hm"], tb, ws.row_group))
                else:
                    ops.linear_fwd(hin, H, Wm.gu, din, A["gu"], 2 * I, T, 2 * I, H, strideB=2 * I * din, **grp)
                    ops.swiglu_fwd_ld_tbl(A["gu"], 2 * I, T, I, p_res, self._seed(l, 4), A["hm"], tb, ws.row_group)
            else:
                ops.rmsnorm_fwd(xcur, W.ln3, eps, A["hin"], din, ws.slot)
                if W.inject:
                    ops.rowtable_fwd(W.beh, r["beh_idx"], A["hin"], din, H, ws.slot)
                if c.fuse_swiglu_fwd and din == H:
                    ops.gemm(A["hin"], din, 1, Wm.gu, din, 1, A["gu"], 2 * I, T, 2 * I, din, strideB=2 * I * din, p_drop=p_res,
                             seed=self._seed(l, 4), swiglu_fwd=(A["hm"], None, None), **grp)
                else:
                    ops.linear_fwd(A["hin"], din, Wm.gu, din, A["gu"], 2 * I, T, 2 * I, din, strideB=2 * I * din, **grp)
                    ops.swiglu_fwd_ld(A["gu"], 2 * I, T, I, p_res, self._seed(l, 4), A["hm"])
            ops.gemm(A["hm"], I, 1, Wm.down, I, 1, xnext, H, T, H, I, strideB=H * I, resid=xcur, row_map=ws.perm,
                     p_drop=p_res, seed=self._seed(l, 5), **grp)
        return self._head(c, x_last if last_row_logits else None, num_items_in_batch, hidden_sink)

    def _route(self, c, actions, act_zero_col, rope_from_mask: bool):
        if rope_from_mask:
            raise ValueError("rope_from_mask is an option of the models without behaviour levels")
        cfg, r, S = self.cfg, c.ws.router, c.S
        act = actions.to(self.device, torch.int64).contiguous() if actions is not None else None
        ops.router_fwd(c.ids, c.am, act, self.lut, cfg.num_positions, cfg.pad_token_id, cfg.eos_token_id, r)
        if self.position_table is not None:
            ops.router_position_table(r["expert"], self.position_table)
        if act_zero_col is None and S % cfg.num_positions == 1:
            act_zero_col = S - 1
        if act_zero_col is not None:
            r["act_idx"][:, act_zero_col] = 0
        return None

    def _shipped_ffn_layer(self, W) -> bool:
        return W.sparse and W.gated and not self.cfg.Moe_behavior_only

    def _ffn_rows(self, l: int):
        return self.ws.slot if self.W[l].sparse else None

    def _ffn_fwd_plain(self, c, l: int, xcur, xnext):
        ws, W, Wm, A = c.ws, self.W[l], self.Wm[l], c.ws.layers[l]
        T, H, I, din, nI = c.T, c.H, c.I, W.din, W.nI
        slot = ws.slot if W.sparse else None
        grp = dict(groups=W.ne, group_offsets=ws.offsets) if W.sparse else {}
        phantom = W.sparse and self.cfg.Moe_behavior_only
        ops.rmsnorm_fwd(xcur, W.ln3, c.eps, A["hin"], din, slot)
        if W.inject:
            ops.rowtable_fwd(W.beh, ws.router["beh_idx"], A["hin"], din, H, slot)
        gu = A["gu"].view(-1)[:T * nI].view(T, nI)
        if phantom:
            gu.zero_()
        ops.linear_fwd(A["hin"], din, Wm.gu, din, gu, nI, T, nI, din, **(dict(strideB=nI * din) if W.sparse else {}), **grp)
        if W.gated:
            ops.swiglu_fwd_ld(gu, nI, T, I, c.p_res, self._seed(l, 4), A["hm"])
        else:
            ops.silu_fwd_ld(gu, nI, T, I, c.p_res, self._seed(l, 4), A["hm"])
        if phantom:
            xnext.copy_(xcur)
        ops.gemm(A["hm"], I, 1, Wm.down, I, 1, xnext, H, T, H, I, resid=xcur, p_drop=c.p_res, seed=self._seed(l, 5),
                 **(dict(strideB=H * I, row_map=ws.perm) if W.sparse else {}), **grp)

    def _ffn_bwd_plain(self, c, l: int, xlast):
        ws, W, G, A = c.ws, self.W[l], self.G[l], c.ws.layers[l]
        WT = self.WT[l] if c.bf16 else None
        T, H, I, din, nI = c.T, c.H, c.I, W.din, W.nI
        t0 = ws.tmpH[0]
        slot = ws.slot if W.sparse else None
        grp = dict(groups=W.ne, group_offsets=ws.offsets) if W.sparse else {}
        sB = (lambda n: dict(strideB=n)) if W.sparse else (lambda n: {})
        sC = (lambda n: dict(strideC=n)) if W.sparse else (lambda n: {})
        if W.sparse and self.cfg.Moe_behavior_only:
            ws.dhm.zero_()
            ws.dhin.zero_()
        with c.hold(t0):
            ops.linear_wgrad(t0, H, A["hm"], I, G.down, I, T, H, I, **sC(H * I), **grp)
            self._dgrad(c, t0, H, W.down, WT.down if c.bf16 else None, I, ws.dhm, I, H, I, **sB(H * I), **grp)
        gu = A["gu"].view(-1)[:T * nI].view(T, nI)
        if W.gated:
            ops.swiglu_bwd_ld(gu, nI, T, I, ws.dhm, c.p_res, self._seed(l, 4))
        else:
            ops.silu_bwd_ld(gu, nI, T, I, ws.dhm, c.p_res, self._seed(l, 4))
        with c.hold(gu):
            ops.linear_wgrad(gu, nI, A["hin"], din, G.gu, din, T, nI, din, **sC(nI * din), **grp)
            self._dgrad(c, gu, nI, W.gu, WT.gu if c.bf16 else None, din, ws.dhin, din, nI, din, **sB(nI * din), **grp)
        if W.inject:
            ops.rowtable_bwd(ws.dhin, din, H, ws.router["beh_idx"], G.beh, slot, partial=ws.norm_partial[-1])
        self._norm_bwd(c, xlast, W.ln3, ws.dhin, din, G.ln3, True, slot,
                       branch=None if W.cross else (self._seed(l, 1), None))

    def ffn_rows(self, W, pos: int, x, beh, out):
        cfg = self.cfg
        B, H, I, din, nI = x.shape[0], cfg.hidden_size, cfg.intermediate_size, W.din, W.nI
        e = cfg.position_experts()[pos] if W.sparse else 0
        if e >= W.ne:
            out.copy_(x)
            return
        f32 = dict(dtype=torch.float32, device=self.device)
        hin = torch.empty(B, din, **f32)
        ops.rmsnorm_fwd(x, W.ln3, float(cfg.rms_norm_eps), hin, din)
        if W.inject:
            ops.rowtable_fwd(W.beh, beh, hin, din, H)
        gu, hm = torch.empty(B, nI, **f32), torch.empty(B, I, **f32)
        ops.linear_fwd(hin, din, W.gu[e * nI:(e + 1) * nI], din, gu, nI, B, nI, din)
        if W.gated:
            ops.swiglu_fwd_ld(gu, nI, B, I, 0.0, 0, hm)
        else:
            ops.silu_fwd_ld(gu, nI, B, I, 0.0, 0, hm)
        ops.gemm(hm, I, 1, W.down[e * H:(e + 1) * H], I, 1, out, H, B, H, I, resid=x)

    def _pass(self, B: int, S: int, p_res: float, p_att: float) -> SimpleNamespace:
        cfg = self.cfg
        c = SimpleNamespace(B=B, S=S, T=B * S, H=cfg.hidden_size, nq=cfg.num_attention_heads, nkv=cfg.num_key_value_heads,
                            dh=cfg.head_dim, I=cfg.intermediate_size, eps=float(cfg.rms_norm_eps), p_res=p_res, p_att=p_att,
                            bf16=self.dtype == "bf16")
        c.NQ, c.NKV = c.nq * c.dh, c.nkv * c.dh
        c.QKV = c.NQ + 2 * c.NKV
        c.scale = float(c.dh) ** -0.5
        c.cos, c.sin = self.rope(S)
        c.split_attn = self.split_attention and self.matmul != "f32" and not c.bf16
        c.h2 = c.split_attn and self.h2_attention and self.matmul == "split3" and p_att < 0.75
        c.fuse_swiglu_fwd = not c.bf16 and self.matmul == "split3" and os.environ.get("GAMER_FUSE_SWIGLU_FWD", "1") != "0"
        c.fuse_swiglu_bwd = (c.bf16 or self.matmul == "split3") and self.fuse_swiglu_bwd
        return c

    def _prologue(self, input_ids, attention_mask, labels, train, dropout, dropout_rate, kv_dest, hidden_sink,
                  last_row_logits, uniform_len, eval_only: Optional[str], f32_only: Optional[str]) -> SimpleNamespace:
        B, S = input_ids.shape
        if kv_dest is not None and train:
            raise ValueError("kv_dest is an evaluation-only option (the backward reads the workspace's q|k|v and keys)")
        if eval_only and (train or labels is not None):
            raise ValueError(eval_only)
        if hidden_sink is not None and last_row_logits:
            raise ValueError("hidden_sink needs the full-sequence forward")
        if self.dtype == "bf16":
            if f32_only:
                raise NotImplementedError(f32_only)
            self.shadow.refresh()
        if self.weight_planes is not None:
            ops.split3_planes(self.flat_p, self.weight_planes)
        use_drop = train if dropout is None else dropout
        c = self._pass(B, S, float(dropout_rate) if use_drop else 0.0,
                       float(self.cfg.attention_dropout) if use_drop else 0.0)
        if use_drop:
            self.dropout_step += 1
        ws = c.ws = self.ws = self.workspace(B, S, train)
        if self._amax is not None:
            self._amax.reset()
            if train:
                self._amax.stable(ws.xn, *[A[k] for A in ws.layers for k in ("h1", "h2", "ao", "ao_c", "hin", "hm") if k in A])
                if self.h2_attention:
                    self._amax.stable(*[A[k] for A in ws.layers for k in ("q", "k", "q_c", "k_c") if k in A],
                                      *[A[k][:, c.NQ + c.NKV:] for A in ws.layers for k in ("qkv", "qkv_c") if k in A])
        c.ids = input_ids.to(self.device, torch.int64).contiguous()
        c.am = attention_mask.to(self.device, torch.int64).contiguous() if attention_mask is not None else None
        c.lab = labels.to(self.device, torch.int64).contiguous() if labels is not None else None
        c.uniform_len, c.train = uniform_len, train
        if c.lab is not None:
            ws.bad_label.zero_()
            ops.check_labels(c.lab, self.cfg.vocab_size, IGNORE_INDEX, ws.bad_label)
        return c

    def _attention(self, c, qb, kb, vb, kl_, ql_, empty_, tile_empty_, seed_, ob, lseb, order_, span_):
        B, S, nq, nkv, NQ, NKV, QKV = c.B, c.S, c.nq, c.nkv, c.NQ, c.NKV, c.QKV
        if c.split_attn and (span_ is None or c.h2):
            ops.attn_fwd_split(qb, NQ, kb, NKV, vb, QKV, kl_, ql_, empty_, B, S, nq, nkv, c.scale, c.p_att, seed_, ob, lseb,
                               order=order_, h2=c.h2, uniform_len=c.uniform_len, q_span=span_)
        elif c.bf16:
            ord16 = (order_[0], order_[2], empty_) if (order_ is not None and span_ is None) else None
            ops.attn_fwd_bf16(qb, NQ, kb, NKV, vb, QKV, kl_, ql_, B, S, nq, nkv, c.scale, c.p_att, seed_, ob, lseb,
                              q_span=span_, order=ord16)
        else:
            ops.attn_fwd(qb, NQ, kb, NKV, vb, QKV, kl_, ql_, empty_, tile_empty_, B, S, nq, nkv, c.scale, c.p_att, seed_,
                         ob, lseb, order=order_, uniform_len=c.uniform_len, q_span=span_)

    def _self_attention(self, c, l: int, masks: dict, span, pos_ids, fuse_qkv: bool, kv_dest, kv_sink):
        W, Wm, A, xs = self.W[l], self.Wm[l], c.ws.layers[l], c.ws.x[l]
        T, H, NQ, NKV, QKV, eps = c.T, c.H, c.NQ, c.NKV, c.QKV, c.eps
        ops.rmsnorm_fwd(xs[0], W.ln1, eps, A["h1"])
        qkv_s, k_s = kv_dest(l, "self") if kv_dest is not None else (A["qkv"], A["k"])
        if fuse_qkv:
            ops.gemm(A["h1"], H, 1, Wm.self_attn["qkv"], H, 1, qkv_s, QKV, T, QKV, H,
                     qknorm=dict(wq=W.self_attn["qn"], wk=W.self_attn["kn"], eps=eps, cos=c.cos, sin=c.sin, q_rot=A["q"],
                                 k_rot=k_s, pos_ids=pos_ids, S=c.S, nq=c.nq, nkv=c.nkv))
        else:
            v_amax = dict(c_amax=(qkv_s[:, NQ + NKV:], NQ + NKV)) if (c.h2 and self.gemm_c_amax) else {}
            ops.linear_fwd(A["h1"], H, Wm.self_attn["qkv"], H, qkv_s, QKV, T, QKV, H, **v_amax)
            ops.qknorm_rope_fwd(qkv_s, c.S, c.nq, c.nkv, W.self_attn["qn"], W.self_attn["kn"], eps, c.cos, c.sin, A["q"], k_s,
                                pos_ids=pos_ids)
        if kv_sink is not None:
            kv_sink(l, "self", k_s, qkv_s[:, NQ + NKV:])
        self._attention(c, A["q"], k_s, qkv_s[:, NQ + NKV:], masks["kl_self"], None, masks["empty_self"],
                        masks["tile_empty_self"], self._seed(l, 0), A["ao"], A["lse"], None, span)
        ops.gemm(A["ao"], NQ, 1, Wm.self_attn["o"], NQ, 1, xs[1], H, T, H, NQ, resid=xs[0], p_drop=c.p_res,
                 seed=self._seed(l, 1))

    def _head(self, c, x_last: Optional[torch.Tensor], num_items_in_batch, hidden_sink):
        ws, B, S, H, eps = c.ws, c.B, c.S, c.H, c.eps
        V = self.cfg.vocab_size
        if x_last is not None:
            xn = torch.empty_like(x_last)
            ops.rmsnorm_fwd(x_last, self.params["model.norm.weight"], eps, xn)
            small = torch.empty(B, ws.ldl, dtype=torch.float32, device=self.device)
            ops.linear_fwd(xn, H, self.params["model.embed_tokens.weight"], H, small, ws.ldl, B, V, H)
            self._saved = None
            self.last_logits_buf = small
            return None, small.view(B, 1, ws.ldl)[:, :, :V]
        ops.rmsnorm_fwd(ws.x_final, self.params["model.norm.weight"], eps, ws.xn)
        if hidden_sink is not None:
            hidden_sink.append(ws.xn.view(B, S, H).clone())
        emb_m = self.shadow.params16["model.embed_tokens.weight"] if c.bf16 else self.params["model.embed_tokens.weight"]
        lab = c.lab
        head_alpha = (1.0 / self.temperature) if (lab is not None and ws.logits.dtype == torch.float32) else 1.0
        ops.linear_fwd(ws.xn, H, emb_m, H, ws.logits, ws.ldl, c.T, V, H, alpha=head_alpha)
        loss = None
        if lab is not None:
            ops.ce_fwd(ws.logits, ws.ldl, lab, V, 1.0 if head_alpha != 1.0 else self.temperature, IGNORE_INDEX, ws.lse_ce,
                       ws.row_loss, ws.loss_sum, ws.count)
            if torch.is_tensor(num_items_in_batch):
                num_items_in_batch = num_items_in_batch.to(self.device, torch.float32).reshape(1)
                loss = ws.loss_sum[0] / num_items_in_batch[0]
            elif num_items_in_batch is not None:
                loss = ws.loss_sum[0] / float(num_items_in_batch)
            else:
                loss = ws.loss_sum[0] / ws.count[0]
        self._saved = dict(ids=c.ids, labels=lab, num_items=num_items_in_batch, train=c.train, p_res=c.p_res, p_att=c.p_att,
                           B=B, S=S, dropout_step=self.dropout_step)
        return loss, ws.logits.view(B, S, ws.ldl)[:, :, :V]

    def check_inputs(self):
        n = int(self.ws.router["bad_token"].item())
        if n:
            raise IndexError(f"{n} item(s) start with a token that is not in config.behavior_maps "
                             "(the reference fails with an embedding IndexError, router.py:170-171)")
        n = int(self.ws.bad_label.item())
        if n:
            raise IndexError(f"{n} label(s) outside [0, vocab_size={self.cfg.vocab_size}) that are not -100 "
                             "(nn.CrossEntropyLoss raises 'Target out of bounds' in the reference)")
        if self.variant == "session" and self.ws.session is not None:
            n = int(self.ws.session["violations"].item())
            if n:
                raise ValueError(f"{n} row(s) with session ids that decrease along the sequence or RoPE positions "
                                 "outside [0, S): the session masks are built as causal key spans "
                                 "(gamer_session_spans), which needs the dataset's layout (SMB_dataset.py:194-222)")

    def zero_grad(self):
        ops.fill(self.flat_g, 0.0)

    @ops.scoped_f32_matmul(lambda self, *a: self.matmul, lambda self, *a: self._planes())
    @ops.scoped_amax(lambda self, *a: self._amax)
    def backward(self, dloss: float = 1.0, layer_done=None, dloss_dev: Optional[torch.Tensor] = None):
        sv = self._saved
        if sv is None or not sv["train"] or sv["labels"] is None:
            raise RuntimeError("backward() needs forward(train=True, labels=...) first")
        with ops.deterministic(True if self.deterministic else ops.DETERMINISTIC_WGRAD, bf16=True if self.deterministic else None):
            return self._backward(dloss, layer_done, dloss_dev)

    def _backward(self, dloss: float = 1.0, layer_done=None, dloss_dev: Optional[torch.Tensor] = None):
        cfg = self.cfg
        c = self._backward_head(dloss, dloss_dev, rows=self._ffn_rows(cfg.num_hidden_layers - 1))
        ws, B, S, T, H, I, E = c.ws, c.B, c.S, c.T, c.H, c.I, cfg.num_experts
        nq, nkv, NQ, NKV, QKV, eps, cos, sin, p_res = c.nq, c.nkv, c.NQ, c.NKV, c.QKV, c.eps, c.cos, c.sin, c.p_res
        NB1 = cfg.num_behavior + 1
        span_self = span_cross = pos_ids = None
        if self.variant == "session":
            span_self, span_cross, pos_ids = ws.session["span_self"], ws.session["span_cross"], ws.session["pos_ids"]
        r = ws.router
        NP = ws.norm_partial[-1]
        hold, fuse_delta, do_amax, fuse_swiglu_bwd = c.hold, c.fuse_delta, c.do_amax, c.fuse_swiglu_bwd
        dgrad, norm_bwd = functools.partial(self._dgrad, c), functools.partial(self._norm_bwd, c)
        attention_bwd = functools.partial(self._attention_bwd, c)
        t0, t1, t2, t3 = ws.tmpH
        bf16 = c.bf16
        for l in reversed(range(cfg.num_hidden_layers)):
            W, G, A, xs = self.W[l], self.G[l], ws.layers[l], ws.x[l]
            WT = self.WT[l] if bf16 else None
            din = W.din
            grp = dict(groups=E, group_offsets=ws.offsets)
            xlast = xs[2] if W.cross else xs[1]
            if not self._shipped_ffn_layer(W):
                self._ffn_bwd_plain(c, l, xlast)
            else:
                split_inj = W.inject and self.split_inject
                tb = ws._buf(f"l{l}_inject_tbl", (E * NB1, 2 * I)) if split_inj else None
                with hold(t0):
                    ops.linear_wgrad(t0, H, A["hm"], I, G.down, I, T, H, I, strideC=H * I, **grp)
                    if fuse_swiglu_bwd and split_inj:
                        ops.gemm(t0, H, 1, W.down, 1, I, ws.dhm, I, T, I, H, strideB=H * I, p_drop=p_res, seed=self._seed(l, 4),
                                 swiglu_bwd=(A["gu"], 2 * I), groups=E * NB1, group_offsets=ws.grp_offsets, group_div=NB1, sw_tbl=tb)
                    elif fuse_swiglu_bwd:
                        if bf16:
                            ops.linear_dgrad_t(t0, H, WT.down, WT.down.shape[1], ws.dhm, I, T, H, I, strideB=H * I, p_drop=p_res,
                                               seed=self._seed(l, 4), swiglu_bwd=(A["gu"], 2 * I), **grp)
                        else:
                            ops.gemm(t0, H, 1, W.down, 1, I, ws.dhm, I, T, I, H, strideB=H * I, p_drop=p_res, seed=self._seed(l, 4),
                                     swiglu_bwd=(A["gu"], 2 * I), **grp)
                    else:
                        dgrad(t0, H, W.down, WT.down if bf16 else None, I, ws.dhm, I, H, I, strideB=H * I, **grp)
                if not fuse_swiglu_bwd:
                    if split_inj:
                        ops.swiglu_bwd_ld_tbl(A["gu"], 2 * I, T, I, ws.dhm, p_res, self._seed(l, 4), tb, ws.row_group)
                    else:
                        ops.swiglu_bwd_ld(A["gu"], 2 * I, T, I, ws.dhm, p_res, self._seed(l, 4))
                if split_inj:
                    hin = A["hin"].view(-1)[:T * H].view(T, H)
                    dhin = ws.dhin.view(-1)[:T * H].view(T, H)
                    with hold(A["gu"]):
                        ops.linear_wgrad(A["gu"], 2 * I, hin, H, G.gu, din, T, 2 * I, H, strideC=2 * I * din, **grp)
                        dgrad(A["gu"], 2 * I, W.gu, None, din, dhin, H, 2 * I, H, strideB=2 * I * din, **grp)
                    seg = ws._buf("inject_segsum", (E * NB1, 2 * I))
                    seg_ws = ws._buf("inject_seg_ws", (ops.segment_colsum_ws_floats(T, 2 * I, E * NB1),))
                    ops.segment_colsum(A["gu"], 2 * I, T, 2 * I, ws.grp_offsets, E * NB1, seg_ws, seg)
                    ops.inject_table_bwd(seg, W.beh, W.gu, din, H, E, 2 * I, G.gu, G.beh,
                                         ws._buf("inject_scratch", (NB1 * E * cfg.behavior_embedding_dim,)))
                    norm_bwd(xlast, W.ln3, dhin, H, G.ln3, True, ws.slot, branch=None if W.cross else (self._seed(l, 1), None))
                else:
                    with hold(A["gu"]):
                        ops.linear_wgrad(A["gu"], 2 * I, A["hin"], din, G.gu, din, T, 2 * I, din, strideC=2 * I * din, **grp)
                        dgrad(A["gu"], 2 * I, W.gu, WT.gu if bf16 else None, din, ws.dhin, din, 2 * I, din, strideB=2 * I * din, **grp)
                    if W.inject:
                        ops.rowtable_bwd(ws.dhin, din, H, r["beh_idx"], G.beh, ws.slot, partial=NP)
                    norm_bwd(xlast, W.ln3, ws.dhin, din, G.ln3, True, ws.slot,
                             branch=None if W.cross else (self._seed(l, 1), None))
            if W.cross:
                C, GC = W.cross_attn, G.cross_attn
                CT = WT.cross_attn if bf16 else dict(o=None, gate=None, qkv=None)
                ops.silu_gate_bwd(A["op_c"], A["gate_c"], ws.dx, t1, t2, p=p_res, seed=self._seed(l, 3))
                hold_t2 = hold(t2)
                hold_t2.__enter__()
                with hold(t1):
                    ops.linear_wgrad(t1, H, A["ao_c"], NQ, GC["o"], NQ, T, H, NQ)
                    ops.linear_wgrad(t2, H, A["h2"], H, GC["gate"], H, T, H, H)
                    dgrad(t1, H, C["o"], CT["o"], NQ, ws.dao, NQ, H, NQ,
                          rowdot=(A["ao_c"], ws.delta, S) if fuse_delta else None, **do_amax)
                attention_bwd(A["q_c"], A["k_c"], A["qkv_c"][:, NQ + NKV:], A["ao_c"], A["lse_c"], r["kl_cross"],
                              r["ql_cross"], r["empty_cross"], r["tile_empty_cross"], self._seed(l, 2), ws.cross_order,
                              span_cross)
                ops.qknorm_rope_bwd(A["qkv_c"], ws.dq, ws.dk, S, nq, nkv, C["qn"], C["kn"], eps, cos, sin, ws.dqkv,
                                    GC["qn"], GC["kn"], bias_q=C["bq"], bias_k=C["bk"], act_idx=r["act_idx"], nb1=NB1,
                                    dbias_q=GC["bq"], dbias_k=GC["bk"], dbias_v=GC["bv"], pos_ids=pos_ids,
                                    partial=ws.qk_partial)
                with hold(ws.dqkv):
                    ops.linear_wgrad(ws.dqkv, QKV, A["h2"], H, GC["qkv"], H, T, QKV, H)
                    dgrad(ws.dqkv, QKV, C["qkv"], CT["qkv"], H, t3, H, QKV, H)
                dgrad(t2, H, C["gate"], CT["gate"], H, t3, H, H, H, accumulate=True)
                hold_t2.__exit__(None, None, None)
                norm_bwd(xs[1], W.ln2, t3, H, G.ln2, True, branch=(self._seed(l, 1), None))
            self._self_attention_bwd(c, l, r, span_self, pos_ids, rows=self._ffn_rows(l - 1) if l > 0 else None)
            if layer_done is not None:
                layer_done(l)
        self._backward_tail(c)

    def _backward_head(self, dloss, dloss_dev, rows) -> SimpleNamespace:
        sv = self._saved
        c = self._pass(sv["B"], sv["S"], sv["p_res"], sv["p_att"])
        ws = c.ws = self.ws
        c.saved_step = self.dropout_step
        self.dropout_step = sv["dropout_step"]
        c.ids, c.norm_dws = sv["ids"], []
        c.fuse_delta = (ws.ds_work is not None or c.bf16 or c.split_attn) and c.T % 128 == 0 and c.NQ % 128 == 0
        c.do_amax = dict(c_amax=(ws.dao, 0)) if (c.h2 and self.gemm_c_amax) else {}
        c.hold = self._amax.hold if self._amax is not None else (lambda *t: contextlib.nullcontext())
        V, H, T, L = self.cfg.vocab_size, c.H, c.T, self.cfg.num_hidden_layers
        if torch.is_tensor(sv["num_items"]):
            ops.ce_bwd(ws.logits, ws.ldl, sv["labels"], V, self.temperature, IGNORE_INDEX, ws.lse_ce, sv["num_items"], 0.0,
                       dloss, dloss_dev)
        elif sv["num_items"] is not None:
# ... 130 lines not shown
```

### gamer_amd/ops.py

```python
from __future__ import annotations

import ctypes as C
from typing import Optional

import os

import torch

from . import _lib
from ._lib import GemmBf16Desc, GemmDesc, call, ptr, stream_ptr


def _sfx(t: torch.Tensor) -> str:
    if t.dtype == torch.float32:
        return ""
    if t.dtype == torch.bfloat16:
        return "_bf16"
    raise RuntimeError(f"activations must be float32 or bfloat16, got {t.dtype}")


def _chk(t: torch.Tensor, dtype, name: str):
    if not t.is_cuda:
        raise RuntimeError(f"{name} must be on the HIP device (gamer_amd has no CPU path)")
    if t.dtype != dtype:
# ... 279 lines not shown
                        if self._ttable is None or self._ttable[0] != live:
                            tab = [v for (p_, b_, r_, c_) in live for i in range(b_) for v in ((p_ - base) // 4 + i * r_ * c_, r_, c_)]
                            self._ttable = (live, torch.tensor(tab, dtype=torch.int64, device=dev), len(tab) // 3)
                        call("gamer_split2h_transpose_multi", self.planes.data_ptr(), self._ttable[1].data_ptr(), self._ttable[2],
                             self.planes_t.data_ptr(), stream_ptr())
                        self._tplane_keys = {(p_, "dense", b_ * r_ * c_) for (p_, b_, r_, c_) in live}

    def register(self, *tensors):
        if not self.stable_ranges:
            return
        b0, n0 = self.stable_ranges[0]
        for t in tensors:
            p, n = t.data_ptr(), t.numel()
            if (b0 <= p and p + 4 * n <= b0 + n0 and n % 4 == 0 and t.is_contiguous() and
                    not any(p_ < p + 4 * n and p < p_ + 4 * n_ for (p_, n_) in self._wkeys)):
                self._wkeys.append((p, n))
                self._wdev = t.device

    def reserve(self, n):
        while len(self.pools) * 1024 - self.used < n and self.pools:
            self.pools.append(torch.zeros(1024 * AMAX_WORDS, dtype=torch.int32, device=self.pools[0].device))

    def register_transposed(self, t, batch, rows, cols):
        if self.planes_t is None or not t.is_contiguous() or t.numel() != batch * rows * cols or rows % 4 or cols % 4:
            return
        key = (t.data_ptr(), int(batch), int(rows), int(cols))
        if key not in self._tkeys:
            self._tkeys.append(key)
            self.register(t)

    def plane_parent(self, p, geom):
        key = self._key(p, geom)
        if key in self._plane_keys or len(key) == 3:
            return None
        batch, stride, rows, cols, ld = geom
        end = p + 4 * ((batch - 1) * stride + (rows - 1) * ld + cols)
        for (p_, kind, n_) in self._plane_keys:
            if p_ <= p and end <= p_ + 4 * n_:
                return self.slots.get((p_, kind, n_))
        return None

    def hold(self, *tensors):
        cache = self

        class _Hold:
            def __enter__(self_h):
                for t in tensors:
                    cache.held[t.data_ptr()] = cache.held.get(t.data_ptr(), 0) + 1

            def __exit__(self_h, *exc):
                for t in tensors:
                    p = t.data_ptr()
                    cache.held[p] -= 1
                    if cache.held[p] == 0:
                        del cache.held[p]
                        for k in [k for k in cache.slots if k[0] == p]:
                            del cache.slots[k]
                return False
        return _Hold()

    def _cached(self, p):
        if self.everything or p in self.stable_ptrs or p in self.held:
            return True
        return any(b <= p < b + n for b, n in self.stable_ranges)

    @staticmethod
    def _key(p, geom):
        batch, stride, rows, cols, ld = geom
        if ld == cols and (batch == 1 or stride == rows * ld):
            return (p, "dense", batch * rows * cols)
        return (p,) + tuple(geom)

    def _new_slot(self, device):
        i, j = divmod(self.used, 1024)
        if i == len(self.pools):
            self.pools.append(torch.zeros(1024 * AMAX_WORDS, dtype=torch.int32, device=device))
        self.used += 1
        return self.pools[i].data_ptr() + 4 * AMAX_WORDS * j

    def preset(self, x, geom, accumulate=False):
        key = self._key(x.data_ptr(), geom)
        if accumulate and key in self.pending:
            return self.pending[key]
        if accumulate == "only":
            return None
        self.slots.pop(key, None)
        ptr_ = self.pending[key] = self._new_slot(x.device)
        return ptr_

    def peek(self, x, geom):
        key = self._key(x.data_ptr(), geom)
        return self.pending.get(key) or self.slots.get(key)

    def slot(self, x, geom):
        p = x.data_ptr()
        key = self._key(p, geom)
        keep = self._cached(p)
        if key in self.pending:
            ptr_ = self.pending.pop(key)
            if keep:
                self.slots[key] = ptr_
            return ptr_
        if keep and key in self.slots:
            return self.slots[key]
        ptr_ = self._new_slot(x.device)
        call("gamer_absmax_f32", ptr(x), *geom, ptr_, stream_ptr())
        if keep:
            self.slots[key] = ptr_
            if (len(key) == 3 and self.stable_ranges and key[2] % 4 == 0 and
                    self.stable_ranges[0][0] <= p < self.stable_ranges[0][0] + self.stable_ranges[0][1] and
                    not any(p_ < p + 4 * key[2] and p < p_ + 4 * n_ for (p_, n_) in self._wkeys)):
                self._wkeys.append((p, key[2]))
                self._wdev = x.device
        return ptr_


def _drop_pending_on_failure(name):
    if _AMAX_REUSE is not None:
        _AMAX_REUSE.pending.clear()


_lib.FAILURE_HOOKS.append(_drop_pending_on_failure)

_AMAX_ATTN = os.environ.get("GAMER_AMAX_ATTN", "1") != "0"


def _arm_sink(*outs):
    if _AMAX_REUSE is None or F32_MATMUL_TERMS != 3 or outs[0][0].dtype != torch.float32:
        return
    slots = [_AMAX_REUSE.preset(t, g, acc) for t, g, acc in outs]
    if slots[0] is None:
        return
    if len(slots) > 2:
        call("gamer_amax_sink3", slots[0], slots[1], slots[2])
    else:
        call("gamer_amax_sink", slots[0], slots[1] if len(slots) > 1 else None)


def scoped_amax(get_cache):
    import functools

    def deco(fn):
        @functools.wraps(fn)
        def wrapper(*args, **kwargs):
            cache = get_cache(*args)
            if cache is None:
                return fn(*args, **kwargs)
            with cache:
                return fn(*args, **kwargs)
        return wrapper
    return deco


def absmax_slot(x, batch, stride, rows, cols, ld):
    if _AMAX_REUSE is not None:
        return _AMAX_REUSE.slot(x, (batch, stride, rows, cols, ld))
    key = (x.device.index, stream_ptr())
    ring = _AMAX_RING.get(key)
    if ring is None:
        ring = _AMAX_RING[key] = [torch.zeros(_AMAX_SLOTS * AMAX_WORDS, dtype=torch.int32, device=x.device), 0]
    if ring[1] == _AMAX_SLOTS:
        ring[0].zero_()
        ring[1] = 0
    slot = ring[0].data_ptr() + 4 * AMAX_WORDS * ring[1]
    ring[1] += 1
    call("gamer_absmax_f32", ptr(x), batch, stride, rows, cols, ld, slot, stream_ptr())
    return slot


def split3_planes(x, planes):
    call("gamer_split3_planes", ptr(x), ptr(planes), x.numel(), planes.stride(0), stream_ptr())


DETERMINISTIC_WGRAD = os.environ.get("GAMER_WGRAD_TWO_PASS", "1") != "0"
DETERMINISTIC_WGRAD_BF16 = os.environ.get("GAMER_WGRAD_TWO_PASS_BF16", "0") == "1"
_WGRAD_WS = {}


class deterministic:

    def __init__(self, on: bool = True, bf16=None):
        self.on, self.bf16 = bool(on), bf16

    def __enter__(self):
        global DETERMINISTIC_WGRAD, DETERMINISTIC_WGRAD_BF16
        self.prev, DETERMINISTIC_WGRAD = DETERMINISTIC_WGRAD, self.on
        self.prev16 = DETERMINISTIC_WGRAD_BF16
        if self.bf16 is not None:
            DETERMINISTIC_WGRAD_BF16 = bool(self.bf16)
        return self

    def __exit__(self, *exc):
        global DETERMINISTIC_WGRAD, DETERMINISTIC_WGRAD_BF16
        DETERMINISTIC_WGRAD, DETERMINISTIC_WGRAD_BF16 = self.prev, self.prev16
        return False


def _wgrad_workspace(device, floats: int) -> torch.Tensor:
    t = _WGRAD_WS.get(device)
    if t is None or t.numel() < floats:
        _WGRAD_WS[device] = None
        t = _WGRAD_WS[device] = torch.empty(int(floats), dtype=torch.float32, device=device)
    return t


class split3_guard:

    def __init__(self, on: bool):
        self.on = bool(on)

    def __enter__(self):
        self.prev = _lib.load().gamer_split3_guard(1 if self.on else 0)
        return self

    def __exit__(self, *exc):
        _lib.load().gamer_split3_guard(self.prev)
        return False


def set_f32_matmul(mode) -> int:
    global F32_MATMUL_TERMS
    prev = F32_MATMUL_TERMS
    terms = MATMUL_MODES[mode] if isinstance(mode, str) else int(mode)
    if terms not in (0, 3, 6, 9):
        raise ValueError(f"fp32 matmul mode {mode!r}: one of {sorted(MATMUL_MODES)}")
    F32_MATMUL_TERMS = terms
    return prev


def gemm(A, a_rs, a_ks, Bm, b_rs, b_ks, Cm, ldc, M, N, K, alpha=1.0, accumulate=False, groups=1, group_mode=0,
         group_offsets=None, strideB=0, strideC=0, kchunk=0, resid=None, row_map=None, p_drop=0.0, seed=0,
         rowdot=None, qknorm=None, c_amax=None, swiglu_bwd=None, group_div=0, sw_tbl=None, swiglu_fwd=None):
    if A.dtype == torch.bfloat16:
        if group_div > 1 or sw_tbl is not None or swiglu_fwd is not None:
            raise RuntimeError("group_div / sw_tbl / swiglu_fwd are options of the fp32 GEMM")
        return _gemm_bf16(A, a_rs, a_ks, Bm, b_rs, b_ks, Cm, ldc, M, N, K, alpha, accumulate, groups, group_mode,
                          group_offsets, strideB, strideC, kchunk, resid, row_map, p_drop, seed, rowdot, qknorm, swiglu_bwd)
    d = GemmDesc()
    d.A = ptr(A); d.a_rs = a_rs; d.a_ks = a_ks
    d.B = ptr(Bm); d.b_rs = b_rs; d.b_ks = b_ks
    d.C = ptr(Cm); d.ldc = ldc
    d.M = M; d.N = N; d.K = K
    d.alpha = alpha
    d.accumulate = 1 if accumulate else 0
    d.groups = groups
    d.group_mode = group_mode
    d.group_offsets = ptr(group_offsets)
    d.strideB = strideB; d.strideC = strideC
    d.kchunk = kchunk
    d.resid = ptr(resid)
    d.row_map = ptr(row_map)
    d.p_drop = p_drop
    d.seed = seed
    if rowdot is not None:
        d.rowdot_other, d.rowdot_out, d.rowdot_S = ptr(rowdot[0]), ptr(rowdot[1]), int(rowdot[2])
    if qknorm is not None:
        q = qknorm
        d.qk_wq, d.qk_wk, d.qk_eps = ptr(q["wq"]), ptr(q["wk"]), float(q["eps"])
        d.qk_cos, d.qk_sin = ptr(q["cos"]), ptr(q["sin"])
        d.qk_bias_q, d.qk_bias_k, d.qk_bias_v = ptr(q.get("bias_q")), ptr(q.get("bias_k")), ptr(q.get("bias_v"))
        d.qk_act_idx, d.qk_pos_ids = ptr(q.get("act_idx")), ptr(q.get("pos_ids"))
        d.qk_q_rot, d.qk_k_rot = ptr(q["q_rot"]), ptr(q["k_rot"])
        d.qk_S, d.qk_nq, d.qk_nkv = int(q["S"]), int(q["nq"]), int(q["nkv"])
    if (c_amax is not None and _AMAX_REUSE is not None and F32_MATMUL_TERMS == 3 and group_mode == 0 and not accumulate
            and resid is None and qknorm is None and c_amax[1] % 64 == 0):
        view, col0 = c_amax
        slot_c = _AMAX_REUSE.preset(view, (1, 0, M, N - col0, ldc))
        d.amax_c, d.amax_c_col0 = slot_c, int(col0)
    if swiglu_bwd is not None:
        gu, ld_gu = swiglu_bwd
        d.sw_gu, d.sw_ld = ptr(gu), int(ld_gu)
        d.sw_tbl = ptr(sw_tbl)
        if _AMAX_REUSE is not None and F32_MATMUL_TERMS == 3 and ld_gu == 2 * N:
            d.amax_c, d.amax_c_col0 = _AMAX_REUSE.preset(gu, (1, 0, 1, M * ld_gu, M * ld_gu)), 0
    d.group_div = int(group_div)
    if swiglu_fwd is not None:
        hm, tbl, row_group = swiglu_fwd
        d.sw_hm, d.sw_tbl, d.sw_row_group = ptr(hm), ptr(tbl), ptr(row_group)
        if _AMAX_REUSE is not None and F32_MATMUL_TERMS == 3:
            d.amax_c, d.amax_c_col0 = _AMAX_REUSE.preset(hm, (1, 0, 1, M * (N // 2), M * (N // 2))), 0
    if group_mode == 1 and DETERMINISTIC_WGRAD:
        n_chunks = (K + kchunk - 1) // kchunk + (groups if group_offsets is not None else 0)
        need = n_chunks * ((M + 127) // 128) * ((N + 127) // 128) * 16384
        ws = _wgrad_workspace(A.device, need)
        d.wgrad_ws, d.wgrad_ws_floats = ws.data_ptr(), ws.numel()
    if F32_MATMUL_TERMS == 3:
        ga = (M, K, a_rs) if a_ks == 1 else (K, M, a_ks)
        gb = (N, K, b_rs) if b_ks == 1 else (K, N, b_ks)
        nb = (groups // max(1, int(group_div))) if (group_mode == 0 and groups > 1) else 1
        d.amax_a = absmax_slot(A, 1, 0, *ga)
        geom_b = (nb, strideB if nb > 1 else 0) + gb
        c = _AMAX_REUSE
        parent = c.plane_parent(Bm.data_ptr(), geom_b) if (c is not None and c.planes is not None and group_mode == 0) else None
        if parent is not None:
            d.amax_b = parent
            d.b_planes = c.planes.data_ptr() + (Bm.data_ptr() - c.stable_ranges[0][0])
            call("gamer_gemm_f32_split", C.byref(d), 3, stream_ptr())
            return
        d.amax_b = absmax_slot(Bm, *geom_b)
        if c is not None and c.planes is not None and group_mode == 0 and c._key(Bm.data_ptr(), geom_b) in c._plane_keys:
            d.b_planes = c.planes.data_ptr() + (Bm.data_ptr() - c.stable_ranges[0][0])
            if a_ks == 1 and b_ks == 1 and c._key(Bm.data_ptr(), geom_b) in c._tplane_keys:
                d.b_planes_t = c.planes_t.data_ptr() + (Bm.data_ptr() - c.stable_ranges[0][0])
        call("gamer_gemm_f32_split", C.byref(d), 3, stream_ptr())
        return
    if F32_MATMUL_TERMS:
        if WEIGHT_PLANES is not None and group_mode == 0:
            base, nbytes, pl, stride = WEIGHT_PLANES
            off = Bm.data_ptr() - base
            if 0 <= off < nbytes:
                d.b_planes, d.b_plane_stride = pl + off // 2, stride
        call("gamer_gemm_f32_split", C.byref(d), F32_MATMUL_TERMS, stream_ptr())
    else:
        call("gamer_gemm_f32", C.byref(d), stream_ptr())


def _gemm_bf16(A, a_rs, a_ks, Bm, b_rs, b_ks, Cm, ldc, M, N, K, alpha, accumulate, groups, group_mode, group_offsets,
               strideB, strideC, kchunk, resid, row_map, p_drop, seed, rowdot, qknorm=None, swiglu_bwd=None):
    if Bm.dtype != torch.bfloat16 or alpha != 1.0:
        raise RuntimeError("gamer_gemm_bf16 takes two bf16 operands and alpha = 1")
    d = GemmBf16Desc()
    if group_mode == 0:
        if a_ks != 1 or b_ks != 1:
            raise RuntimeError("bf16 GEMM: both operands must be k-contiguous (dgrad runs on the transposed weight copy)")
        d.lda, d.ldb = a_rs, b_rs
        want = torch.float32 if resid is not None else torch.bfloat16
    else:
        if a_rs != 1 or b_rs != 1:
            raise RuntimeError("bf16 wgrad: both operands must be token-major")
        d.lda, d.ldb = a_ks, b_ks
        want = torch.float32
    if Cm.dtype != want:
        raise RuntimeError(f"bf16 GEMM: C must be {want}, got {Cm.dtype}")
    d.A, d.B, d.C, d.ldc = ptr(A), ptr(Bm), ptr(Cm), ldc
    d.M, d.N, d.K = M, N, K
    d.accumulate = 1 if accumulate else 0
    d.groups, d.group_mode, d.group_offsets = groups, group_mode, ptr(group_offsets)
    d.strideB, d.strideC, d.kchunk = strideB, strideC, kchunk
    d.resid, d.row_map, d.p_drop, d.seed = ptr(resid), ptr(row_map), p_drop, seed
    if rowdot is not None:
        d.rowdot_other, d.rowdot_out, d.rowdot_S = ptr(rowdot[0]), ptr(rowdot[1]), int(rowdot[2])
    if qknorm is not None:
        q = qknorm
        d.qk_wq, d.qk_wk, d.qk_eps = ptr(q["wq"]), ptr(q["wk"]), float(q["eps"])
        d.qk_cos, d.qk_sin = ptr(q["cos"]), ptr(q["sin"])
        d.qk_bias_q, d.qk_bias_k, d.qk_bias_v = ptr(q.get("bias_q")), ptr(q.get("bias_k")), ptr(q.get("bias_v"))
        d.qk_act_idx, d.qk_pos_ids = ptr(q.get("act_idx")), ptr(q.get("pos_ids"))
        d.qk_q_rot, d.qk_k_rot = ptr(q["q_rot"]), ptr(q["k_rot"])
        d.qk_S, d.qk_nq, d.qk_nkv = int(q["S"]), int(q["nq"]), int(q["nkv"])
    if swiglu_bwd is not None:
        d.sw_gu, d.sw_ld = ptr(swiglu_bwd[0]), int(swiglu_bwd[1])
    if group_mode == 1 and DETERMINISTIC_WGRAD_BF16:
        n_chunks = (K + kchunk - 1) // kchunk + (groups if group_offsets is not None else 0)
        need = n_chunks * ((M + 127) // 128) * ((N + 127) // 128) * 16384
        ws = _wgrad_workspace(A.device, need)
        d.wgrad_ws, d.wgrad_ws_floats = ws.data_ptr(), ws.numel()
    call("gamer_gemm_bf16", C.byref(d), stream_ptr())


def linear_dgrad_t(dy, lddy, WT, ldwt, dx, lddx, M, K_out, N_in, accumulate=False, **grp):
    gemm(dy, lddy, 1, WT, ldwt, 1, dx, lddx, M, N_in, K_out, accumulate=accumulate, **grp)


def qkv_fused_ok(x, M: int, N: int) -> bool:
    return x.dtype in (torch.float32, torch.bfloat16) and M % 128 == 0 and N % 128 == 0


def linear_fwd(x, ldx, W, ldw, y, ldy, M, N, K, accumulate=False, **grp):
    gemm(x, ldx, 1, W, ldw, 1, y, ldy, M, N, K, accumulate=accumulate, **grp)


def linear_dgrad(dy, lddy, W, ldw, dx, lddx, M, N_out, K_in, accumulate=False, **grp):
    gemm(dy, lddy, 1, W, 1, ldw, dx, lddx, M, K_in, N_out, accumulate=accumulate, **grp)


def pick_kchunk(rows: int, grouped: bool) -> int:
    chunk = 1024 if grouped else 2048
    while chunk > 256 and rows < 64 * chunk:
        chunk //= 2
    return chunk


_WGRAD_TUNED = {}
_WGRAD_TUNE = os.environ.get("GAMER_WGRAD_TUNE", "1") != "0"


def _tune_allowed() -> bool:
    if not _WGRAD_TUNE:
        return False
    try:
        import torch.distributed as dist
        if dist.is_available() and dist.is_initialized() and dist.get_world_size() > 1:
            return False
    except Exception:
        pass
    return int(os.environ.get("WORLD_SIZE", "1")) <= 1
_WGRAD_TUNE_FILE = os.environ.get("GAMER_WGRAD_TUNE_FILE", "")


def _tune_key_str(key) -> str:
    return "|".join(str(k) for k in key)


_WGRAD_SHIPPED = os.path.join(os.path.dirname(os.path.abspath(__file__)), "wgrad_chunks.json")


def _load_tune_file():
    import json
    out = {}
    for path in (_WGRAD_SHIPPED, _WGRAD_TUNE_FILE):
        if path == _WGRAD_SHIPPED and os.environ.get("GAMER_WGRAD_IGNORE_SHIPPED", "0") not in ("", "0"):
            continue
        if path and os.path.exists(path):
            try:
                with open(path) as f:
                    out.update({k: int(v) for k, v in json.load(f).items()})
            except (OSError, ValueError):
                pass
    return out


def _save_tune_file():
    import json
    import tempfile
    try:
        d = os.path.dirname(os.path.abspath(_WGRAD_TUNE_FILE))
        fd, tmp = tempfile.mkstemp(prefix=".wgrad_tune.", dir=d)
        with os.fdopen(fd, "w") as f:
            json.dump(_WGRAD_FILE_CACHE, f, indent=0)
        os.replace(tmp, _WGRAD_TUNE_FILE)
    except OSError:
        pass


_WGRAD_FILE_CACHE = _load_tune_file()


def _rule_kchunk(dy, rows, N_out, K_in, groups):
    if dy.dtype == torch.bfloat16:
        tiles = ((N_out + 127) // 128) * ((K_in + 127) // 128)
        per_group = max(1, rows // max(groups, 1))
        chunks = max(1, 512 // (tiles * max(groups, 1)))
        kchunk = min(16384, max(256, -(-per_group // chunks)))
# ... 1112 lines not shown
```

### include/gamer_hip.h

```cpp
#ifndef GAMER_HIP_H
#define GAMER_HIP_H

#include <stdint.h>

#ifdef __cplusplus
extern "C" {
#endif

#define GAMER_ABI_VERSION 9
#define GAMER_AMAX_WORDS 256

typedef uint16_t gamer_bf16;

int gamer_abi_version(void);
const char* gamer_last_error(void);
int gamer_reload_env(void);

int gamer_router_fwd(const int64_t* ids, const int64_t* attn_mask, const int64_t* actions,
                     const int32_t* behavior_lut, int vocab, int B, int S, int num_positions,
                     int pad_id, int eos_id,
                     int32_t* expert, int32_t* beh_idx, int32_t* act_idx,
                     int32_t* kl_self, int32_t* kl_cross, int32_t* ql_cross,
                     int32_t* empty_self, int32_t* empty_cross,
                     int32_t* tile_empty_self, int32_t* tile_empty_cross,
                     int32_t* bad_token, void* stream);

int gamer_session_spans(const int64_t* session_ids, const int64_t* extended_session_ids,
                        const int64_t* attn_mask, const int32_t* kl_cross, const int32_t* ql_cross,
                        int B, int S, int num_positions, int n_rope_positions,
                        int32_t* span_self, int32_t* span_cross, int32_t* pos_ids,
                        int32_t* empty_self, int32_t* empty_cross,
                        int32_t* tile_empty_self, int32_t* tile_empty_cross, int32_t* violations,
                        void* stream);

int gamer_session_prep(const int64_t* session_ids, const int64_t* extended_session_ids, const int64_t* attn_mask,
                       int B, int S, int num_positions, int n_rope_positions, int32_t* kl_self, int32_t* span_self,
                       int32_t* pos_ids, int32_t* empty_self, int32_t* tile_empty_self, int32_t* violations,
                       void* stream);

int gamer_causal_prep(const int64_t* attn_mask, int B, int S, int32_t* kl_self, int32_t* empty_self,
                      int32_t* tile_empty_self, int32_t* pos_ids, int32_t* next_pos, void* stream);

int gamer_moe_router_prep(const int64_t* ids, const int64_t* attn_mask, const int32_t* behavior_lut, int vocab,
                          const int32_t* position_table, int B, int S, int num_positions, int n_items,
                          int use_behavior_token, int pad_id, int eos_id, int32_t* expert, int32_t* beh_idx,
                          int32_t* kl_self, int32_t* empty_self, int32_t* tile_empty_self, int32_t* pos_ids,
                          int32_t* next_pos, int32_t* bad_token, void* stream);

int gamer_expert_lists(const int32_t* expert, int B, int S, int num_experts,
                       int32_t* perm, int32_t* slot, int32_t* offsets, int32_t* work, void* stream);
int gamer_router_position_table(int32_t* expert, int64_t n, const int32_t* table, int n_table, void* stream);

int gamer_embedding_fwd(const int64_t* ids, const float* W, int V, int T, int H, float* x, void* stream);
int gamer_embedding_bwd(const int64_t* ids, const float* dx, int V, int T, int H, int pad_id, float* dW,
                        void* stream);
int64_t gamer_embedding_bwd_ordered_ws_bytes(int V, int T, int H);
int gamer_embedding_bwd_ordered(const int64_t* ids, const float* dx, int V, int T, int H, int pad_id, float* dW,
                                void* ws, int64_t ws_bytes, void* stream);

int gamer_rmsnorm_fwd(const float* x, const float* w, int T, int H, float eps,
                      const int32_t* dst_rows, float* y, int ldy, void* stream);
int gamer_rmsnorm_bwd(const float* x, const float* w, const float* dy, int lddy,
                      const int32_t* dy_rows, int T, int H, float eps, int accumulate_dx,
                      float* dx, float* dw_partial, int n_partial,
                      float* mask_out, const int32_t* mask_rows, float p_drop, uint64_t seed, void* stream);
int gamer_rmsnorm_fwd_bf16(const float* x, const float* w, int T, int H, float eps,
                           const int32_t* dst_rows, gamer_bf16* y, int ldy, void* stream);
int gamer_rmsnorm_bwd_bf16(const float* x, const float* w, const gamer_bf16* dy, int lddy,
                           const int32_t* dy_rows, int T, int H, float eps, int accumulate_dx,
                           float* dx, float* dw_partial, int n_partial,
                           gamer_bf16* mask_out, const int32_t* mask_rows, float p_drop, uint64_t seed, void* stream);
int gamer_colsum_reduce(const float* partial, int rows, int cols, int accumulate, float* out,
                        void* stream);
int gamer_colsum_reduce_batched(const float* partial, int64_t stride, int rows, int cols, int n, float* const* outs,
                                int accumulate, void* stream);

int gamer_rowtable_fwd(const float* table, const int32_t* idx, const int32_t* dst_rows, int T, int E,
                       float* y, int ldy, int col0, void* stream);
int gamer_rowtable_bwd(const float* dy, int lddy, int col0, const int32_t* idx,
                       const int32_t* dy_rows, int T, int E, int n_rows_table, float* dtable,
                       float* partial, int64_t partial_numel, void* stream);
int gamer_rowtable_fwd_bf16(const float* table, const int32_t* idx, const int32_t* dst_rows, int T, int E,
                            gamer_bf16* y, int ldy, int col0, void* stream);
int gamer_rowtable_bwd_bf16(const gamer_bf16* dy, int lddy, int col0, const int32_t* idx,
                            const int32_t* dy_rows, int T, int E, int n_rows_table, float* dtable,
                            float* partial, int64_t partial_numel, void* stream);

typedef struct {
    const float* A; int64_t a_rs, a_ks;
    const float* B; int64_t b_rs, b_ks;
    float* C; int64_t ldc;
    int M, N, K;
    float alpha;
    int accumulate;
    int groups;
    int group_mode;
    const int32_t* group_offsets;
    int64_t strideB, strideC;
    int kchunk;
    const float* resid;
    const int32_t* row_map;
    float p_drop;
    uint64_t seed;
    const float* rowdot_other;
    float* rowdot_out;
    int rowdot_S;
    const float* qk_wq; const float* qk_wk;
    float qk_eps;
    const float* qk_cos; const float* qk_sin;
    const float* qk_bias_q; const float* qk_bias_k; const float* qk_bias_v;
    const int32_t* qk_act_idx;
    const int32_t* qk_pos_ids;
    float* qk_q_rot; float* qk_k_rot;
    int qk_S, qk_nq, qk_nkv;
    const gamer_bf16* b_planes;
    int64_t b_plane_stride;
    const uint32_t* amax_a;
    const uint32_t* amax_b;
    uint32_t* amax_c;
    int amax_c_col0;
    float* wgrad_ws;
    int64_t wgrad_ws_floats;
    float* sw_gu;
    int64_t sw_ld;
    int group_div;
    const float* sw_tbl;
    const gamer_bf16* b_planes_t;
    float* sw_hm;
    const int32_t* sw_row_group;
} gamer_gemm_desc;

int gamer_gemm_f32(const gamer_gemm_desc* d, void* stream);
int gamer_split2h_transpose_multi(const gamer_bf16* planes, const int64_t* table, int n, gamer_bf16* planes_t, void* stream);

int gamer_gemm_f32_split(const gamer_gemm_desc* d, int terms, void* stream);
int gamer_split3_guard(int on);
int gamer_absmax_f32(const float* x, int batch, int64_t stride, int rows, int cols, int64_t ld, uint32_t* out, void* stream);
int gamer_absmax_multi_f32(const float* base, const int64_t* table, int n, uint32_t* out, void* stream);
int gamer_split2h_planes_multi(const float* base, const int64_t* table, int n, const uint32_t* slots, gamer_bf16* planes,
                               void* stream);
int gamer_amax_sink(uint32_t* out0, uint32_t* out1);
int gamer_amax_sink3(uint32_t* out0, uint32_t* out1, uint32_t* out2);
int gamer_attn_split_amax(const uint32_t* q, const uint32_t* k, const uint32_t* v, const uint32_t* d_o);
int gamer_split3_planes(const float* x, gamer_bf16* planes, int64_t n, int64_t plane_stride, void* stream);

typedef struct {
    const gamer_bf16* A; int64_t lda;
    const gamer_bf16* B; int64_t ldb;
    void* C; int64_t ldc;
    int M, N, K;
    int accumulate;
    int groups;
    int group_mode;
    const int32_t* group_offsets;
    int64_t strideB, strideC;
    int kchunk;
    const float* resid;
    const int32_t* row_map;
    float p_drop;
    uint64_t seed;
    const gamer_bf16* rowdot_other;
    float* rowdot_out;
    int rowdot_S;
    const float* qk_wq; const float* qk_wk; float qk_eps;
    const float* qk_cos; const float* qk_sin;
    const float* qk_bias_q; const float* qk_bias_k; const float* qk_bias_v;
    const int32_t* qk_act_idx; const int32_t* qk_pos_ids;
    gamer_bf16* qk_q_rot; gamer_bf16* qk_k_rot;
    int qk_S, qk_nq, qk_nkv;
    gamer_bf16* sw_gu;
    int64_t sw_ld;
    float* wgrad_ws;
    int64_t wgrad_ws_floats;
} gamer_gemm_bf16_desc;

int gamer_gemm_bf16(const gamer_gemm_bf16_desc* d, void* stream);

int gamer_cast_params_bf16(const float* flat, gamer_bf16* out, gamer_bf16* out_t, const int64_t* table,
                           int n_entries, int n_tiles, void* stream);

int gamer_qknorm_rope_fwd(float* qkv, int T, int S, int nq, int nkv,
                          const float* wq, const float* wk, float eps,
                          const float* cos_t, const float* sin_t,
                          const float* bias_q, const float* bias_k, const float* bias_v,
                          const int32_t* act_idx,
                          float* q_rot, float* k_rot, const int32_t* pos_ids, void* stream);
int gamer_qknorm_rope_bwd(const float* qkv, const float* dq_rot, const float* dk_rot,
                          int T, int S, int nq, int nkv,
                          const float* wq, const float* wk, float eps,
                          const float* cos_t, const float* sin_t,
                          const float* bias_q, const float* bias_k,
                          const int32_t* act_idx, int nb1,
                          float* dqkv, float* dwq, float* dwk,
                          float* dbias_q, float* dbias_k, float* dbias_v, const int32_t* pos_ids,
                          float* partial, int64_t partial_numel, void* stream);
int gamer_qknorm_rope_fwd_bf16(gamer_bf16* qkv, int T, int S, int nq, int nkv,
                               const float* wq, const float* wk, float eps,
                               const float* cos_t, const float* sin_t,
                               const float* bias_q, const float* bias_k, const float* bias_v,
                               const int32_t* act_idx,
                               gamer_bf16* q_rot, gamer_bf16* k_rot, const int32_t* pos_ids, void* stream);
int gamer_qknorm_rope_bwd_bf16(const gamer_bf16* qkv, const gamer_bf16* dq_rot, const gamer_bf16* dk_rot,
                               int T, int S, int nq, int nkv,
                               const float* wq, const float* wk, float eps,
                               const float* cos_t, const float* sin_t,
                               const float* bias_q, const float* bias_k,
                               const int32_t* act_idx, int nb1,
                               gamer_bf16* dqkv, float* dwq, float* dwk,
                               float* dbias_q, float* dbias_k, float* dbias_v, const int32_t* pos_ids,
                               float* partial, int64_t partial_numel, void* stream);

int gamer_attn_row_order(const int32_t* row_empty, int B, int S, int32_t* perm, int32_t* tile_kind,
                         int32_t* tile_maxpos, void* stream);
int gamer_attn_fwd(const float* q, int ldq, const float* k, int ldk, const float* v, int ldv,
                   const int32_t* kl, const int32_t* ql, const int32_t* row_empty,
                   const int32_t* tile_empty,
                   int B, int S, int nq, int nkv, float scale, float p_drop, uint64_t seed,
                   float* o, float* lse, const int32_t* row_perm, const int32_t* tile_kind,
                   const int32_t* tile_maxpos, int uniform_len, const int32_t* q_span, void* stream);
int gamer_attn_bwd(const float* q, int ldq, const float* k, int ldk, const float* v, int ldv,
                   const float* o, const float* d_o, const float* lse,
                   const int32_t* kl, const int32_t* ql, const int32_t* row_empty,
                   const int32_t* tile_empty,
                   int B, int S, int nq, int nkv, float scale, float p_drop, uint64_t seed,
                   float* delta, float* dq, int lddq, float* dk, int lddk, float* dv, int lddv,
                   const int32_t* row_perm, const int32_t* tile_kind, const int32_t* tile_maxpos,
                   float* ds_work, const int32_t* q_span, int delta_ready, void* stream);

int gamer_attn_fwd_split(const float* q, int ldq, const float* k, int ldk, const float* v, int ldv,
                         const int32_t* kl, const int32_t* ql, const int32_t* row_empty,
                         int B, int S, int nq, int nkv, float scale, float p_drop, uint64_t seed,
                         float* o, float* lse,
                         const int32_t* row_perm, const int32_t* tile_kind, const int32_t* tile_maxpos,
                         int uniform_len, const int32_t* q_span, void* stream);
int gamer_attn_bwd_split(const float* q, int ldq, const float* k, int ldk, const float* v, int ldv,
                         const float* o, const float* d_o, const float* lse,
                         const int32_t* kl, const int32_t* ql, const int32_t* row_empty, const int32_t* tile_empty,
                         int B, int S, int nq, int nkv, float scale, float p_drop, uint64_t seed,
                         float* delta, float* dq, int lddq, float* dk, int lddk, float* dv, int lddv,
                         const int32_t* row_perm, const int32_t* tile_kind, const int32_t* tile_maxpos,
                         int delta_ready, float* ds_work, const int32_t* q_span, void* stream);

int gamer_attn_fwd_bf16(const gamer_bf16* q, int ldq, const gamer_bf16* k, int ldk, const gamer_bf16* v, int ldv,
                        const int32_t* kl, const int32_t* ql, int B, int S, int nq, int nkv, float scale,
                        float p_drop, uint64_t seed, gamer_bf16* o, float* lse, const int32_t* q_span,
                        const int32_t* row_perm, const int32_t* tile_maxpos, const int32_t* row_empty, void* stream);
int gamer_attn_bwd_bf16(const gamer_bf16* q, int ldq, const gamer_bf16* k, int ldk, const gamer_bf16* v, int ldv,
                        const gamer_bf16* o, const gamer_bf16* d_o, const float* lse, const int32_t* kl,
                        const int32_t* ql, int B, int S, int nq, int nkv, float scale, float p_drop, uint64_t seed,
                        float* delta, gamer_bf16* dq, int lddq, gamer_bf16* dk, int lddk, gamer_bf16* dv, int lddv,
                        const int32_t* q_span, int delta_ready, const int32_t* row_perm, const int32_t* tile_maxpos,
                        const int32_t* row_empty, void* stream);

int gamer_bias_act_fwd(float* x, const float* bias, int T, int N, int act, float* y, void* stream);
int gamer_bias_act_bwd(const float* pre, const float* dy, int T, int N, int act, float* dx,
                       float* db_partial, int n_partial, void* stream);
int gamer_layernorm_fwd(const float* x, const float* res, const float* w, const float* b, int T, int H,
                        float eps, float* v_out, float* y, float* mean, float* rstd, void* stream);
int gamer_layernorm_bwd(const float* v, const float* w, const float* mean, const float* rstd,
                        const float* dy, int T, int H, float* dx, float* dw_partial, float* db_partial,
                        int n_partial, void* stream);
int gamer_attn_dense_fwd(const float* q, int ldq, const float* k, int ldk, const float* v, int ldv,
                         const float* mask, const int64_t* mask_strides, int B, int S, int H, int head_dim,
                         float scale, float p_drop, uint64_t seed, float* o, int ldo, float* lse, void* stream);
int gamer_attn_dense_bwd(const float* q, int ldq, const float* k, int ldk, const float* v, int ldv,
                         const float* mask, const int64_t* mask_strides, int B, int S, int H, int head_dim,
                         float scale, float p_drop, uint64_t seed, const float* o, const float* d_o, int ldo,
                         const float* lse, float* dq, int lddq, float* dk, int lddk, float* dv, int lddv,
                         void* stream);

int gamer_residual_dropout_fwd(const float* x_in, const float* delta, const int32_t* src_rows, int T,
                               int H, float p_drop, uint64_t seed, float* x_out, void* stream);
int gamer_residual_dropout_bwd(const float* dx, const int32_t* src_rows, int T, int H,
                               float p_drop, uint64_t seed, float* ddelta, void* stream);
int gamer_swiglu_fwd(const float* g, const float* u, int64_t n, float p_drop, uint64_t seed,
                     float* hm, void* stream);
int gamer_swiglu_bwd(float* g, float* u, const float* dhm, int64_t n, float p_drop, uint64_t seed,
                     void* stream);
int gamer_swiglu_fwd_ld(const float* gu, int64_t ld, int T, int I, float p_drop, uint64_t seed, float* hm, void* stream);
int gamer_swiglu_bwd_ld(float* gu, int64_t ld, int T, int I, const float* dhm, float p_drop, uint64_t seed, void* stream);
int gamer_swiglu_fwd_ld_tbl(const float* gu, int64_t ld, int T, int I, float p_drop, uint64_t seed, float* hm,
                            const float* tbl, const int32_t* row_group, void* stream);
// ... 204 lines not shown
```

Measured before the change: 5086.

## Fuse RMSNorm prologue and per-row bias epilogue into activation-stationary split GEMM

```diff
diff --git a/gamer_amd/_lib.py b/gamer_amd/_lib.py
--- a/gamer_amd/_lib.py
+++ b/gamer_amd/_lib.py
@@ -53,6 +53,10 @@
         ("sw_gu", c_void_p), ("sw_ld", c_int64),
         ("group_div", c_int), ("sw_tbl", c_void_p), ("b_planes_t", c_void_p),
         ("sw_hm", c_void_p), ("sw_row_group", c_void_p),
+        ("norm_x", c_void_p), ("norm_w", c_void_p), ("norm_eps", c_float),
+        ("norm_dst_rows", c_void_p), ("norm_src_rows", c_void_p),
+        ("bias_idx", c_void_p), ("bias_q", c_void_p), ("bias_k", c_void_p), ("bias_v", c_void_p),
+        ("bias_rows", c_int), ("bias_nq", c_int), ("bias_nkv", c_int),
     ]
 
 
diff --git a/gamer_amd/csrc/common.h b/gamer_amd/csrc/common.h
--- a/gamer_amd/csrc/common.h
+++ b/gamer_amd/csrc/common.h
@@ -305,6 +305,7 @@
 
 bool gemm_as_eligible(const gamer_gemm_desc* d, bool a_kc, bool b_kc, const uint16_t* b_planes);
 int launch_gemm_as(const gamer_gemm_desc* d, const uint16_t* b_planes, bool b_kc, hipStream_t st);
+int launch_gemm_bias_rows(const gamer_gemm_desc* d, hipStream_t st);
 bool gemm_os_eligible(const gamer_gemm_desc* d, bool a_kc, bool b_kc, const uint16_t* b_planes);
 int launch_gemm_os(const gamer_gemm_desc* d, const uint16_t* b_planes, int guard, hipStream_t st, bool fwd_t = false);
 bool gemm_os_fwd_eligible(const gamer_gemm_desc* d, bool a_kc, bool b_kc);
diff --git a/gamer_amd/csrc/gemm.hip b/gamer_amd/csrc/gemm.hip
--- a/gamer_amd/csrc/gemm.hip
+++ b/gamer_amd/csrc/gemm.hip
@@ -1388,7 +1388,31 @@
                                   aligned16(d->C) && (!d->sw_tbl || d->sw_row_group) && d->p_drop >= 0.f && d->p_drop < 1.f),
                     "gamer_gemm_f32: the SwiGLU-forward epilogue (sw_hm) needs a Linear-forward layout with N = 2 I (N=%d), alpha = 1, no other "
                     "epilogue, and sw_row_group with sw_tbl", d->N);
+    GAMER_CHECK_ARG(!d->norm_x || (d->norm_w && d->group_mode == 0 && a_kc && b_kc && d->norm_eps > 0.f && d->K % 4 == 0 && d->K <= 1024 &&
+                                   aligned16(d->norm_x) && aligned16(d->norm_w) &&
+                                   (d->norm_dst_rows != nullptr) == (d->norm_src_rows != nullptr)),
+                    "gamer_gemm_f32: the RMSNorm prologue (norm_x) needs a Linear-forward layout, norm_w, norm_eps > 0, K %% 4 == 0 (K=%d) "
+                    "and norm_dst_rows / norm_src_rows both or neither", d->K);
+    GAMER_CHECK_ARG(!d->bias_idx || (d->bias_q && d->bias_k && d->bias_v && d->group_mode == 0 && d->groups == 1 && a_kc && b_kc &&
+                                     !d->accumulate && !d->resid && !d->rowdot_out && !d->qk_q_rot && !d->sw_gu && !d->sw_hm &&
+                                     d->bias_rows >= 1 && d->bias_nq > 0 && d->bias_nkv > 0 && d->bias_nq % 4 == 0 && d->bias_nkv % 4 == 0 &&
+                                     d->N == d->bias_nq + 2 * d->bias_nkv && d->ldc % 4 == 0 && aligned16(d->C) && aligned16(d->bias_q) &&
+                                     aligned16(d->bias_k) && aligned16(d->bias_v)),
+                    "gamer_gemm_f32: the bias-row epilogue (bias_idx) needs a plain Linear-forward GEMM with one group, three tables and "
+                    "N = bias_nq + 2 bias_nkv in multiples of 4 (N=%d)", d->N);
     if (split == 3 && gemm_as_eligible(d, a_kc, b_kc, p.b_planes)) return launch_gemm_as(d, p.b_planes, b_kc, (hipStream_t)stream);
+    if (d->norm_x || d->bias_idx) {
+        gamer_gemm_desc d2 = *d;
+        if (d->norm_x) {
+            if (d->amax_a) gamer_amax_sink(const_cast<uint32_t*>(d->amax_a), nullptr);
+            GAMER_TRY(gamer_rmsnorm_fwd(d->norm_x, d->norm_w, d->M, d->K, d->norm_eps, d->norm_dst_rows, const_cast<float*>(d->A), (int)d->a_rs,
+                                        stream));
+            d2.norm_x = nullptr; d2.norm_w = nullptr; d2.norm_dst_rows = nullptr; d2.norm_src_rows = nullptr;
+        }
+        if (d->bias_idx) { d2.bias_idx = nullptr; d2.amax_c = nullptr; }
+        GAMER_TRY(gemm_entry(&d2, stream, split));
+        return d->bias_idx ? launch_gemm_bias_rows(d, (hipStream_t)stream) : 0;
+    }
     if (d->sw_hm) {
         gamer_gemm_desc d2 = *d;
         d2.sw_hm = nullptr; d2.sw_row_group = nullptr; d2.sw_tbl = nullptr; d2.amax_c = nullptr;
diff --git a/gamer_amd/csrc/gemm_as.hip b/gamer_amd/csrc/gemm_as.hip
--- a/gamer_amd/csrc/gemm_as.hip
+++ b/gamer_amd/csrc/gemm_as.hip
@@ -39,11 +39,15 @@
     const float* rowdot_other; float* rowdot_out; int rowdot_S;
     float* sw_gu; int64_t sw_ld; float p_drop; uint64_t seed;
     float* hm; const float* tbl; int group_div;
+    const float* norm_w; float norm_eps; float* h; int64_t ldh; const int32_t* src_rows; uint32_t* amax_h;
+    const int32_t* act_idx; const float* bias_q; const float* bias_k; const float* bias_v; int bias_c1, bias_c2, nb1;
 };
 
-template <int KP, bool WRC, int EPI, int NW>
+template <int KP, bool WRC, int EPI, int NW, bool NORM = false, bool BIAS = false>
 __global__ void __launch_bounds__(64 * NW, AS_DEPTH == 2 ? 1 : 8 / NW)
 gemm_as_kernel(const AsParams p) {
+    static_assert(!(NORM || BIAS) || !WRC, "the norm prologue and the bias epilogue are built for W k-contiguous");
+    static_assert(!BIAS || EPI == 0, "the bias epilogue belongs to the plain store");
     constexpr int AS_WAVES_K = NW, AS_THREADS_K = 64 * NW;
     extern __shared__ __attribute__((aligned(16))) unsigned char as_raw[];
     bf16_t* const wimg = reinterpret_cast<bf16_t*>(as_raw);
@@ -72,13 +76,35 @@
     bf16x8 af[2][KP * 4];
     float row_inv;
     {
-        const float* arow = p.A + (int64_t)(valid_m ? m : row_end - 1) * p.lda + 8 * h;
+        int64_t src_row = valid_m ? m : row_end - 1;
+        if (NORM && p.src_rows) src_row = p.src_rows[src_row];
+        const float* arow = p.A + src_row * p.lda + 8 * h;
         float4 raw[KP * 8];
 #pragma unroll
         for (int s = 0; s < KP * 4; ++s) {
             raw[2 * s] = *reinterpret_cast<const float4*>(arow + 16 * s);
             raw[2 * s + 1] = *reinterpret_cast<const float4*>(arow + 16 * s + 4);
         }
+        if constexpr (NORM) {
+            float ss = 0.f;
+#pragma unroll
+            for (int i = 0; i < KP * 8; ++i) ss += raw[i].x * raw[i].x + raw[i].y * raw[i].y + raw[i].z * raw[i].z + raw[i].w * raw[i].w;
+            ss = xor32_sum(ss);
+            const float rstd = rsqrtf(ss * (1.f / (float)(KP * 64)) + p.norm_eps);
+            float* hrow = p.h + (int64_t)m * p.ldh + 8 * h;
+            const float* wrow = p.norm_w + 8 * h;
+#pragma unroll
+            for (int s = 0; s < KP * 4; ++s) {
+#pragma unroll
+                for (int j = 0; j < 2; ++j) {
+                    const float4 w4 = *reinterpret_cast<const float4*>(wrow + 16 * s + 4 * j);
+                    float4 x = raw[2 * s + j];
+                    x.x = w4.x * (x.x * rstd); x.y = w4.y * (x.y * rstd); x.z = w4.z * (x.z * rstd); x.w = w4.w * (x.w * rstd);
+                    raw[2 * s + j] = x;
+                    if (valid_m) *reinterpret_cast<float4*>(hrow + 16 * s + 4 * j) = x;
+                }
+            }
+        }
         float mx = 0.f;
 #pragma unroll
         for (int i = 0; i < KP * 8; ++i) {
@@ -86,6 +112,14 @@
             mx = fmaxf(fmaxf(fmaxf(mx, fabsf(raw[i].x)), fabsf(raw[i].y)), fmaxf(fabsf(raw[i].z), fabsf(raw[i].w)));
         }
         mx = xor32_max(mx);
+        if constexpr (NORM) {
+            if (p.amax_h) {
+                uint32_t hm = __float_as_uint(mx);
+#pragma unroll
+                for (int o2 = 16; o2 > 0; o2 >>= 1) hm = max(hm, (uint32_t)__shfl_xor((int)hm, o2, 64));
+                if (lane == 0 && hm) amax_publish(hm, p.amax_h, blockIdx.x * AS_WAVES_K + w);
+            }
+        }
         float s_row = 1.f;
         row_inv = 1.f;
         if (mx > 0.f) scale_from_amax(__float_as_uint(mx), s_row, row_inv);
@@ -170,6 +204,18 @@
     if (EPI == 5 && p.tbl) {
         const float4* src = reinterpret_cast<const float4*>(p.tbl + (int64_t)grp * p.N);
         for (int i = tid; i < p.N / 4; i += AS_THREADS_K) reinterpret_cast<float4*>(tbl_lds)[i] = src[i];
+    }
+    int bias_row = 0;
+    if constexpr (BIAS) {
+        const int n4 = p.N >> 2;
+        for (int i = tid; i < p.nb1 * n4; i += AS_THREADS_K) {
+            const int a = i / n4, c = 4 * (i - a * n4);
+            const float* src = c < p.bias_c1 ? p.bias_q + (int64_t)a * p.bias_c1 + c
+                             : c < p.bias_c2 ? p.bias_k + (int64_t)a * (p.bias_c2 - p.bias_c1) + (c - p.bias_c1)
+                                             : p.bias_v + (int64_t)a * (p.N - p.bias_c2) + (c - p.bias_c2);
+            reinterpret_cast<float4*>(tbl_lds)[i] = *reinterpret_cast<const float4*>(src);
+        }
+        if (valid_m) bias_row = min(max(p.act_idx[m], 0), p.nb1 - 1) * p.N;
     }
 
     float cmax = 0.f;
@@ -214,6 +260,11 @@
                             float4 t4 = make_float4(acc[nt][4 * g4] * out_scale, acc[nt][4 * g4 + 1] * out_scale,
                                                     acc[nt][4 * g4 + 2] * out_scale, acc[nt][4 * g4 + 3] * out_scale);
                             if (AS_ABLATE & 1) { asm volatile("" :: "v"(t4.x), "v"(t4.y), "v"(t4.z), "v"(t4.w)); continue; }
+                            if constexpr (BIAS) {
+                                asm volatile("" : "+v"(t4.x), "+v"(t4.y), "+v"(t4.z), "+v"(t4.w));
+                                const float4 b4 = *reinterpret_cast<const float4*>(tbl_lds + bias_row + col);
+                                t4.x += b4.x; t4.y += b4.y; t4.z += b4.z; t4.w += b4.w;
+                            }
                             if (EPI == 4) {
                                 float* ga = p.sw_gu + (int64_t)m * p.sw_ld + col;
                                 const float4 a4 = *reinterpret_cast<const float4*>(ga), b4 = *reinterpret_cast<const float4*>(ga + p.N);
@@ -328,6 +379,7 @@
 }
 
 static std::atomic<long long> g_as_launches{0};
+static std::atomic<long long> g_as_fused_launches{0};
 
 static inline bool gemm_as_enabled() {
     static EnvSwitch sw("GAMER_GEMM_AS");
@@ -338,6 +390,18 @@
     if (!gemm_as_enabled() || !a_kc || !b_planes || !d->amax_b) return false;
     if (d->group_mode != 0 || d->resid || d->qk_q_rot) return false;
     if ((d->group_div > 1 || d->sw_tbl) && !d->sw_hm) return false;
+    if (d->norm_x) {
+        static EnvSwitch swn("GAMER_GEMM_AS_NORM");
+        if (swn.get(1) == 0 || !b_kc || !d->norm_w || !aligned16(d->norm_x) || !aligned16(d->norm_w) || !aligned16(d->A) ||
+            (d->norm_dst_rows != nullptr) != (d->norm_src_rows != nullptr))
+            return false;
+    }
+    if (d->bias_idx) {
+        static EnvSwitch swb("GAMER_GEMM_AS_BIAS");
+        if (swb.get(1) == 0 || !b_kc || d->sw_hm || d->groups != 1 || d->accumulate || d->bias_rows < 1 ||
+            (int64_t)d->bias_rows * d->N * (int64_t)sizeof(float) > 16384)
+            return false;
+    }
     if (d->sw_hm) {
         static EnvSwitch sw5("GAMER_GEMM_AS_SWIGLU");
         if (sw5.get(1) == 0 || !b_kc || d->accumulate || d->rowdot_out || d->sw_gu || d->N % (2 * AS_SLAB) != 0 || d->alpha != 1.f ||
@@ -372,10 +436,17 @@
 template <int KP, bool WRC, int EPI>
 static int launch_as(int nw, dim3 grid, size_t shmem, hipStream_t st, const AsParams& p) {
     const char* who = "gamer_gemm_f32_split/activation-stationary";
-    if constexpr (EPI == 5) return launch<gemm_as_kernel<KP, WRC, EPI, 4>>(who, grid, dim3(64 * 4), shmem, st, p);
-    else
+    [[maybe_unused]] const bool norm = p.norm_w != nullptr, bias = p.act_idx != nullptr;
+    if constexpr (WRC) {
         return with_flags([&](auto eight) { return launch<gemm_as_kernel<KP, WRC, EPI, eight() ? 8 : 4>>(who, grid, dim3(eight() ? 512 : 256), shmem, st, p); },
                           nw == 8);
+    } else if constexpr (EPI == 5) {
+        return with_flags([&](auto nm) { return launch<gemm_as_kernel<KP, WRC, EPI, 4, nm()>>(who, grid, dim3(64 * 4), shmem, st, p); }, norm);
+    } else {
+        return with_flags([&](auto eight, auto nm, auto bs) {
+            return launch<gemm_as_kernel<KP, WRC, EPI, eight() ? 8 : 4, nm(), bs()>>(who, grid, dim3(eight() ? 512 : 256), shmem, st, p); },
+                          nw == 8, norm, bias);
+    }
 }
 
 int launch_gemm_as(const gamer_gemm_desc* d, const uint16_t* b_planes, bool b_kc, hipStream_t st) {
@@ -392,8 +463,15 @@
     p.rowdot_other = d->rowdot_other; p.rowdot_out = d->rowdot_out; p.rowdot_S = d->rowdot_S;
     p.sw_gu = d->sw_gu; p.sw_ld = d->sw_ld; p.p_drop = d->p_drop; p.seed = d->seed;
     p.hm = d->sw_hm; p.tbl = d->sw_hm ? d->sw_tbl : nullptr; p.group_div = d->group_div > 1 ? d->group_div : 1;
+    const bool norm = b_kc && d->norm_x, bias = b_kc && d->bias_idx;
+    p.norm_w = norm ? d->norm_w : nullptr; p.norm_eps = d->norm_eps; p.src_rows = norm ? d->norm_src_rows : nullptr;
+    p.h = const_cast<float*>(d->A); p.ldh = d->a_rs; p.amax_h = norm ? const_cast<uint32_t*>(d->amax_a) : nullptr;
+    if (norm) { p.A = d->norm_x; p.lda = d->K; }
+    p.act_idx = bias ? d->bias_idx : nullptr; p.bias_q = d->bias_q; p.bias_k = d->bias_k; p.bias_v = d->bias_v;
+    p.bias_c1 = d->bias_nq; p.bias_c2 = d->bias_nq + d->bias_nkv; p.nb1 = d->bias_rows;
     const int kp = d->K / 64;
-    const size_t shmem = (size_t)(AS_DEPTH == 2 ? 3 : 2) * 2 * kp * AS_PANEL * sizeof(bf16_t) + (d->sw_hm ? (size_t)d->N * sizeof(float) : 0);
+    const size_t shmem = (size_t)(AS_DEPTH == 2 ? 3 : 2) * 2 * kp * AS_PANEL * sizeof(bf16_t) + (d->sw_hm ? (size_t)d->N * sizeof(float) : 0) +
+                         (bias ? (size_t)d->bias_rows * d->N * sizeof(float) : 0);
     static EnvSwitch wv("GAMER_GEMM_AS_WAVES");
     const int nw = d->sw_hm ? 4 : (wv.is_set() ? (wv.get(4) == 8 ? 8 : 4) : ((b_kc && d->groups == 1 && d->N >= 512 && AS_WAVES == 4) ? 8 : AS_WAVES));
     const dim3 grid((d->M + 32 * nw - 1) / (32 * nw) + (p.group_offsets ? d->groups : 0));
@@ -421,9 +499,41 @@
     }
     if (rc) return rc;
     g_as_launches.fetch_add(1, std::memory_order_relaxed);
+    if (norm || bias) g_as_fused_launches.fetch_add(1, std::memory_order_relaxed);
     return 0;
 }
 
+__global__ void __launch_bounds__(256)
+gemm_bias_rows_kernel(float* __restrict__ Cm, int64_t ldc, int M, int N, const int32_t* __restrict__ idx, const float* __restrict__ bq,
+                      const float* __restrict__ bk, const float* __restrict__ bv, int c1, int c2, int nb1, uint32_t* __restrict__ amax_c,
+                      int col0) {
+    __shared__ uint32_t amax_lds[4];
+    uint32_t am = 0;
+    const int n4 = N >> 2;
+    const int64_t total = (int64_t)M * n4;
+    for (int64_t i = (int64_t)blockIdx.x * 256 + threadIdx.x; i < total; i += (int64_t)gridDim.x * 256) {
+        const int m = (int)(i / n4), c = 4 * (int)(i - (int64_t)m * n4);
+        const int a = min(max(idx[m], 0), nb1 - 1);
+        const float* src = c < c1 ? bq + (int64_t)a * c1 + c : c < c2 ? bk + (int64_t)a * (c2 - c1) + (c - c1) : bv + (int64_t)a * (N - c2) + (c - c2);
+        const float4 b4 = *reinterpret_cast<const float4*>(src);
+        float4* dst = reinterpret_cast<float4*>(Cm + (int64_t)m * ldc + c);
+        float4 x = *dst;
+        x.x += b4.x; x.y += b4.y; x.z += b4.z; x.w += b4.w;
+        *dst = x;
+        if (c >= col0) am = amax_f4(am, x);
+    }
+    amax_block_commit(am, amax_c, amax_lds);
+}
+
+int launch_gemm_bias_rows(const gamer_gemm_desc* d, hipStream_t st) {
+    const int64_t total = (int64_t)d->M * (d->N >> 2);
+    const int blocks = total > 8192 * 256 ? 8192 : (int)((total + 255) / 256);
+    return launch<gemm_bias_rows_kernel>("gamer_gemm_f32/bias rows", dim3(blocks), dim3(256), 0, st, d->C, d->ldc, d->M, d->N, d->bias_idx,
+                                         d->bias_q, d->bias_k, d->bias_v, d->bias_nq, d->bias_nq + d->bias_nkv, d->bias_rows, d->amax_c,
+                                         d->amax_c_col0);
+}
+
 }
 
 extern "C" long long gamer_debug_gemm_as_launches(void) { return gamer::g_as_launches.load(std::memory_order_relaxed); }
+extern "C" long long gamer_debug_gemm_as_fused_launches(void) { return gamer::g_as_fused_launches.load(std::memory_order_relaxed); }
diff --git a/gamer_amd/engine.py b/gamer_amd/engine.py
--- a/gamer_amd/engine.py
+++ b/gamer_amd/engine.py
@@ -567,7 +567,10 @@
             xcur = xs[1]
             if W.cross:
                 C, Cm = W.cross_attn, Wm.cross_attn
-                ops.rmsnorm_fwd(xs[1], W.ln2, eps, A["h2"])
+                nrm = dict(norm=dict(x=xs[1], w=W.ln2, eps=eps)) if (c.fuse_norm and not fuse_qkv) else {}
+                fuse_bias = c.fuse_bias and not fuse_qkv
+                if not nrm:
+                    ops.rmsnorm_fwd(xs[1], W.ln2, eps, A["h2"])
                 qkv_x, k_x = kv_dest(l, "cross") if kv_dest is not None else (A["qkv_c"], A["k_c"])
                 h2_hold = self._amax.hold(A["h2"]) if (self._amax is not None and not train) else None
                 if h2_hold is not None:
@@ -577,8 +580,13 @@
                              qknorm=dict(wq=C["qn"], wk=C["kn"], eps=eps, cos=cos, sin=sin, q_rot=A["q_c"], k_rot=k_x,
                                          bias_q=C["bq"], bias_k=C["bk"], bias_v=C["bv"], act_idx=r["act_idx"],
                                          pos_ids=pos_ids, S=S, nq=nq, nkv=nkv))
+                elif fuse_bias:
+                    ops.linear_fwd(A["h2"], H, Cm["qkv"], H, qkv_x, QKV, T, QKV, H,
+                                   bias=dict(idx=r["act_idx"], q=C["bq"], k=C["bk"], v=C["bv"]),
+                                   c_amax=(qkv_x[:, NQ + NKV:], NQ + NKV), **nrm)
+                    ops.qknorm_rope_fwd(qkv_x, S, nq, nkv, C["qn"], C["kn"], eps, cos, sin, A["q_c"], k_x, pos_ids=pos_ids)
                 else:
-                    ops.linear_fwd(A["h2"], H, Cm["qkv"], H, qkv_x, QKV, T, QKV, H)
+                    ops.linear_fwd(A["h2"], H, Cm["qkv"], H, qkv_x, QKV, T, QKV, H, **nrm)
                     ops.qknorm_rope_fwd(qkv_x, S, nq, nkv, C["qn"], C["kn"], eps, cos, sin, A["q_c"], k_x,
                                         bias_q=C["bq"], bias_k=C["bk"], bias_v=C["bv"], act_idx=r["act_idx"],
                                         pos_ids=pos_ids)
@@ -625,27 +633,32 @@
                 self._ffn_fwd_plain(c, l, xcur, xnext)
                 continue
             grp = dict(groups=E, group_offsets=ws.offsets)
+            nrm = dict(norm=dict(x=xcur, w=W.ln3, eps=eps, dst_rows=ws.slot, src_rows=ws.perm)) if c.fuse_norm else {}
             if W.inject and self.split_inject:
                 hin = A["hin"].view(-1)[:T * H].view(T, H)
-                ops.rmsnorm_fwd(xcur, W.ln3, eps, hin, H, ws.slot)
+                if not nrm:
+                    ops.rmsnorm_fwd(xcur, W.ln3, eps, hin, H, ws.slot)
                 tb = ws._buf((f"l{l}_" if train else "l_") + "inject_tbl", (E * NB1, 2 * I))
                 ops.inject_table_fwd(W.beh, W.gu, din, H, E, 2 * I, tb)
                 if c.fuse_swiglu_fwd:
                     ops.gemm(hin, H, 1, Wm.gu, din, 1, A["gu"], 2 * I, T, 2 * I, H, strideB=2 * I * din, groups=E * NB1,
                              group_offsets=ws.grp_offsets, group_div=NB1, p_drop=p_res, seed=self._seed(l, 4),
-                             swiglu_fwd=(A["hm"], tb, ws.row_group))
+                             swiglu_fwd=(A["hm"], tb, ws.row_group), **nrm)
                 else:
-                    ops.linear_fwd(hin, H, Wm.gu, din, A["gu"], 2 * I, T, 2 * I, H, strideB=2 * I * din, **grp)
+                    ops.linear_fwd(hin, H, Wm.gu, din, A["gu"], 2 * I, T, 2 * I, H, strideB=2 * I * din, **grp, **nrm)
                     ops.swiglu_fwd_ld_tbl(A["gu"], 2 * I, T, I, p_res, self._seed(l, 4), A["hm"], tb, ws.row_group)
             else:
-                ops.rmsnorm_fwd(xcur, W.ln3, eps, A["hin"], din, ws.slot)
+                if din != H:
+                    nrm = {}
+                if not nrm:
+                    ops.rmsnorm_fwd(xcur, W.ln3, eps, A["hin"], din, ws.slot)
                 if W.inject:
                     ops.rowtable_fwd(W.beh, r["beh_idx"], A["hin"], din, H, ws.slot)
                 if c.fuse_swiglu_fwd and din == H:
                     ops.gemm(A["hin"], din, 1, Wm.gu, din, 1, A["gu"], 2 * I, T, 2 * I, din, strideB=2 * I * din, p_drop=p_res,
-                             seed=self._seed(l, 4), swiglu_fwd=(A["hm"], None, None), **grp)
+                             seed=self._seed(l, 4), swiglu_fwd=(A["hm"], None, None), **grp, **nrm)
                 else:
-                    ops.linear_fwd(A["hin"], din, Wm.gu, din, A["gu"], 2 * I, T, 2 * I, din, strideB=2 * I * din, **grp)
+                    ops.linear_fwd(A["hin"], din, Wm.gu, din, A["gu"], 2 * I, T, 2 * I, din, strideB=2 * I * din, **grp, **nrm)
                     ops.swiglu_fwd_ld(A["gu"], 2 * I, T, I, p_res, self._seed(l, 4), A["hm"])
             ops.gemm(A["hm"], I, 1, Wm.down, I, 1, xnext, H, T, H, I, strideB=H * I, resid=xcur, row_map=ws.perm,
                      p_drop=p_res, seed=self._seed(l, 5), **grp)
@@ -754,6 +767,8 @@
         c.h2 = c.split_attn and self.h2_attention and self.matmul == "split3" and p_att < 0.75
         c.fuse_swiglu_fwd = not c.bf16 and self.matmul == "split3" and os.environ.get("GAMER_FUSE_SWIGLU_FWD", "1") != "0"
         c.fuse_swiglu_bwd = (c.bf16 or self.matmul == "split3") and self.fuse_swiglu_bwd
+        c.fuse_norm = not c.bf16 and self.matmul == "split3" and os.environ.get("GAMER_GEMM_AS_NORM", "1") != "0"
+        c.fuse_bias = not c.bf16 and self.matmul == "split3" and os.environ.get("GAMER_GEMM_AS_BIAS", "1") != "0"
         return c
 
     def _prologue(self, input_ids, attention_mask, labels, train, dropout, dropout_rate, kv_dest, hidden_sink,
@@ -809,7 +824,9 @@
     def _self_attention(self, c, l: int, masks: dict, span, pos_ids, fuse_qkv: bool, kv_dest, kv_sink):
         W, Wm, A, xs = self.W[l], self.Wm[l], c.ws.layers[l], c.ws.x[l]
         T, H, NQ, NKV, QKV, eps = c.T, c.H, c.NQ, c.NKV, c.QKV, c.eps
-        ops.rmsnorm_fwd(xs[0], W.ln1, eps, A["h1"])
+        nrm = dict(norm=dict(x=xs[0], w=W.ln1, eps=eps)) if (c.fuse_norm and not fuse_qkv) else {}
+        if not nrm:
+            ops.rmsnorm_fwd(xs[0], W.ln1, eps, A["h1"])
         qkv_s, k_s = kv_dest(l, "self") if kv_dest is not None else (A["qkv"], A["k"])
         if fuse_qkv:
             ops.gemm(A["h1"], H, 1, Wm.self_attn["qkv"], H, 1, qkv_s, QKV, T, QKV, H,
@@ -817,7 +834,7 @@
                                  k_rot=k_s, pos_ids=pos_ids, S=c.S, nq=c.nq, nkv=c.nkv))
         else:
             v_amax = dict(c_amax=(qkv_s[:, NQ + NKV:], NQ + NKV)) if (c.h2 and self.gemm_c_amax) else {}
-            ops.linear_fwd(A["h1"], H, Wm.self_attn["qkv"], H, qkv_s, QKV, T, QKV, H, **v_amax)
+            ops.linear_fwd(A["h1"], H, Wm.self_attn["qkv"], H, qkv_s, QKV, T, QKV, H, **v_amax, **nrm)
             ops.qknorm_rope_fwd(qkv_s, c.S, c.nq, c.nkv, W.self_attn["qn"], W.self_attn["kn"], eps, c.cos, c.sin, A["q"], k_s,
                                 pos_ids=pos_ids)
         if kv_sink is not None:
@@ -838,13 +855,15 @@
             self._saved = None
             self.last_logits_buf = small
             return None, small.view(B, 1, ws.ldl)[:, :, :V]
-        ops.rmsnorm_fwd(ws.x_final, self.params["model.norm.weight"], eps, ws.xn)
-        if hidden_sink is not None:
-            hidden_sink.append(ws.xn.view(B, S, H).clone())
+        nrm = dict(norm=dict(x=ws.x_final, w=self.params["model.norm.weight"], eps=eps)) if c.fuse_norm else {}
+        if not nrm:
+            ops.rmsnorm_fwd(ws.x_final, self.params["model.norm.weight"], eps, ws.xn)
         emb_m = self.shadow.params16["model.embed_tokens.weight"] if c.bf16 else self.params["model.embed_tokens.weight"]
         lab = c.lab
         head_alpha = (1.0 / self.temperature) if (lab is not None and ws.logits.dtype == torch.float32) else 1.0
-        ops.linear_fwd(ws.xn, H, emb_m, H, ws.logits, ws.ldl, c.T, V, H, alpha=head_alpha)
+        ops.linear_fwd(ws.xn, H, emb_m, H, ws.logits, ws.ldl, c.T, V, H, alpha=head_alpha, **nrm)
+        if hidden_sink is not None:
+            hidden_sink.append(ws.xn.view(B, S, H).clone())
         loss = None
         if lab is not None:
             ops.ce_fwd(ws.logits, ws.ldl, lab, V, 1.0 if head_alpha != 1.0 else self.temperature, IGNORE_INDEX, ws.lse_ce,
diff --git a/gamer_amd/ops.py b/gamer_amd/ops.py
--- a/gamer_amd/ops.py
+++ b/gamer_amd/ops.py
@@ -455,8 +455,10 @@
     return deco
 
 
-def absmax_slot(x, batch, stride, rows, cols, ld):
+def absmax_slot(x, batch, stride, rows, cols, ld, produced=False):
     if _AMAX_REUSE is not None:
+        if produced:
+            _AMAX_REUSE.preset(x, (batch, stride, rows, cols, ld))
         return _AMAX_REUSE.slot(x, (batch, stride, rows, cols, ld))
     key = (x.device.index, stream_ptr())
     ring = _AMAX_RING.get(key)
@@ -467,7 +469,8 @@
         ring[1] = 0
     slot = ring[0].data_ptr() + 4 * AMAX_WORDS * ring[1]
     ring[1] += 1
-    call("gamer_absmax_f32", ptr(x), batch, stride, rows, cols, ld, slot, stream_ptr())
+    if not produced:
+        call("gamer_absmax_f32", ptr(x), batch, stride, rows, cols, ld, slot, stream_ptr())
     return slot
 
 
@@ -533,10 +536,10 @@
 
 def gemm(A, a_rs, a_ks, Bm, b_rs, b_ks, Cm, ldc, M, N, K, alpha=1.0, accumulate=False, groups=1, group_mode=0,
          group_offsets=None, strideB=0, strideC=0, kchunk=0, resid=None, row_map=None, p_drop=0.0, seed=0,
-         rowdot=None, qknorm=None, c_amax=None, swiglu_bwd=None, group_div=0, sw_tbl=None, swiglu_fwd=None):
+         rowdot=None, qknorm=None, c_amax=None, swiglu_bwd=None, group_div=0, sw_tbl=None, swiglu_fwd=None, norm=None, bias=None):
     if A.dtype == torch.bfloat16:
-        if group_div > 1 or sw_tbl is not None or swiglu_fwd is not None:
-            raise RuntimeError("group_div / sw_tbl / swiglu_fwd are options of the fp32 GEMM")
+        if group_div > 1 or sw_tbl is not None or swiglu_fwd is not None or norm is not None or bias is not None:
+            raise RuntimeError("group_div / sw_tbl / swiglu_fwd / norm / bias are options of the fp32 GEMM")
         return _gemm_bf16(A, a_rs, a_ks, Bm, b_rs, b_ks, Cm, ldc, M, N, K, alpha, accumulate, groups, group_mode,
                           group_offsets, strideB, strideC, kchunk, resid, row_map, p_drop, seed, rowdot, qknorm, swiglu_bwd)
     d = GemmDesc()
@@ -577,6 +580,15 @@
         if _AMAX_REUSE is not None and F32_MATMUL_TERMS == 3 and ld_gu == 2 * N:
             d.amax_c, d.amax_c_col0 = _AMAX_REUSE.preset(gu, (1, 0, 1, M * ld_gu, M * ld_gu)), 0
     d.group_div = int(group_div)
+    if norm is not None:
+        nx = norm["x"]
+        if group_mode != 0 or a_ks != 1 or b_ks != 1 or nx.dim() != 2 or nx.shape[0] < M or nx.shape[1] != K or not nx.is_contiguous():
+            raise RuntimeError("gemm(norm=...): a Linear-forward GEMM whose rows are the RMSNorm of a dense [M, K] tensor")
+        d.norm_x, d.norm_w, d.norm_eps = ptr(norm["x"]), ptr(norm["w"]), float(norm["eps"])
+        d.norm_dst_rows, d.norm_src_rows = ptr(norm.get("dst_rows")), ptr(norm.get("src_rows"))
+    if bias is not None:
+        d.bias_idx, d.bias_q, d.bias_k, d.bias_v = ptr(bias["idx"]), ptr(bias["q"]), ptr(bias["k"]), ptr(bias["v"])
+        d.bias_rows, d.bias_nq, d.bias_nkv = int(bias["q"].shape[0]), int(bias["q"].shape[1]), int(bias["k"].shape[1])
     if swiglu_fwd is not None:
         hm, tbl, row_group = swiglu_fwd
         d.sw_hm, d.sw_tbl, d.sw_row_group = ptr(hm), ptr(tbl), ptr(row_group)
@@ -591,7 +603,7 @@
         ga = (M, K, a_rs) if a_ks == 1 else (K, M, a_ks)
         gb = (N, K, b_rs) if b_ks == 1 else (K, N, b_ks)
         nb = (groups // max(1, int(group_div))) if (group_mode == 0 and groups > 1) else 1
-        d.amax_a = absmax_slot(A, 1, 0, *ga)
+        d.amax_a = absmax_slot(A, 1, 0, *ga, produced=norm is not None)
         geom_b = (nb, strideB if nb > 1 else 0) + gb
         c = _AMAX_REUSE
         parent = c.plane_parent(Bm.data_ptr(), geom_b) if (c is not None and c.planes is not None and group_mode == 0) else None
diff --git a/include/gamer_hip.h b/include/gamer_hip.h
--- a/include/gamer_hip.h
+++ b/include/gamer_hip.h
@@ -128,6 +128,14 @@
     const gamer_bf16* b_planes_t;
     float* sw_hm;
     const int32_t* sw_row_group;
+    const float* norm_x;
+    const float* norm_w;
+    float norm_eps;
+    const int32_t* norm_dst_rows;
+    const int32_t* norm_src_rows;
+    const int32_t* bias_idx;
+    const float* bias_q; const float* bias_k; const float* bias_v;
+    int bias_rows, bias_nq, bias_nkv;
 } gamer_gemm_desc;
 
 int gamer_gemm_f32(const gamer_gemm_desc* d, void* stream);
```

After: 5138, median of 6. +1.0%, better.
